# lawfuyang/HobbyRenderer

Hardware: AMD Instinct MI355X
Metric: Mrays/s at 1920×1080, 8 spp, 4 bounces; 1/2/4/8 GPU scaling (higher is better)
Workload: dtype f32; 1 GPU; config 2: Cornell-box-class procedural scene (38 triangles, 9 instances, closed room, emissive quad + default sun), 1920x1080, 8 spp (accumulation indices 0..7), 4 bounces; frames_in_flight=2, serial_kernels=False, mode=default

## Files before the change

hobbyrenderer_amd/csrc/pt_capi.cpp:

```cpp
#include <hip/hip_runtime.h>

#include <chrono>
#include <cstdio>
#include <cstdlib>
#include <cstring>
#include <mutex>
#include <new>
#include <stdexcept>
#include <limits>
#include <string>
#include <system_error>
#include <thread>
#include <vector>

#include "../../include/hobbyrt_pt.h"
#include "bvh_build.h"
#include "bvh_build_gpu.h"
#include "pt_device.h"
#include "pt_kernels.h"
#include "pt_motion.h"
#include "pt_wavefront.h"

using namespace hrt;

// ... 6 lines not shown
    std::vector<void*> bvhAllocations;
    GpuNodeQ* nodesQ = nullptr; size_t nodesQCapacity = 0;
    uint32_t nodes4Capacity = 0;
    GpuBvhBuilder* gpuBuilder = nullptr;
    GpuBvhBuilder* tlasBuilder = nullptr; uint32_t tlasBuilderInstances = 0;
    std::vector<HrptVertexQuantized> keptVertices; std::vector<uint32_t> keptIndices; std::vector<HrptMeshData> keptMeshData;
    std::vector<HrptPerInstanceData> keptInstances; std::vector<HrptMaterialConstants> keptMaterials; std::vector<HrptGPULight> keptLights;
    size_t lightCapacity = 0;
    SceneView view{};
    bool haveScene = false;
    uint32_t bvhNodes = 0, bvhTris = 0;
    uint32_t width = 0, height = 0;
    float4* dAccum = nullptr; float4* dOutput = nullptr; float4* dDisplay = nullptr;
    uint32_t* dHistogram = nullptr; float* dExposure = nullptr;
    uint32_t* dBloomDown = nullptr; uint32_t* dBloomUp = nullptr; size_t bloomWords = 0;
    uint32_t bloomTailTexels = 0;
    float4* dGBuffer[HRPT_GB_PLANES] = {};
    float4* dMotion = nullptr;
    MotionInst* dMotionInst = nullptr; size_t motionInstCapacity = 0;
    float* dMotionPositions = nullptr; uint32_t* dMotionIndices = nullptr;
    bool motionInstStale = true, motionGeometryStale = true;
    float4* dTemporal[2] = {}; int temporalCur = 0; bool temporalValid = false;
    float* dDenoiseTile = nullptr; float4* dDenoiseScratch[2] = {};
    DeviceCounters* dCounters = nullptr;
    hipEvent_t evStart = nullptr, evStop = nullptr;
    bool timed = false;
    WavefrontState wf;
    SceneTraits traits;
    int bvhBuilder = HRPT_BVH_BUILDER_AUTO;
    int accelStructure = HRPT_ACCEL_AUTO;
    BuiltTwoLevel* twoLevel = nullptr;
    std::vector<void*> meshAllocations;
    uint32_t megakernelFallbacks = 0;
    HrptBuildInfo buildInfo{};
};

static std::mutex g_errMutex;
static std::string g_createError;

static int fail(HrptContext* ctx, int code, const std::string& msg)
{
    if (ctx) ctx->err = msg;
    else { std::lock_guard<std::mutex> l(g_errMutex); g_createError = msg; }
    return code;
}
#define HIP_TRY(ctx, expr)                                                                         \
    do {                                                                                           \
        hipError_t e_ = (expr);                                                                    \
        if (e_ != hipSuccess) return fail(ctx, e_ == hipErrorOutOfMemory ? HRPT_ERR_OUT_OF_MEMORY : HRPT_ERR_HIP, \
                                          std::string(#expr) + ": " + hipGetErrorString(e_));      \
    } while (0)

static uint16_t float_to_half(float f)
{
    uint32_t x; memcpy(&x, &f, 4);
    uint32_t sign = (x >> 16) & 0x8000u;
    x &= 0x7fffffffu;
    if (x >= 0x47800000u) return (uint16_t)(sign | 0x7c00u | ((x > 0x7f800000u) ? (0x200u | ((x >> 13) & 0x3ffu)) : 0u));
    if (x < 0x38800000u) {
        if (x < 0x33000000u) return (uint16_t)sign;
        uint32_t shift = 126u - (x >> 23);
        uint32_t m = (x & 0x7fffffu) | 0x800000u;
        uint32_t h = m >> shift, rem = m & ((1u << shift) - 1u), halfway = 1u << (shift - 1u);
        if (rem > halfway || (rem == halfway && (h & 1u))) ++h;
        return (uint16_t)(sign | h);
    }
    uint32_t r = x + 0xfffu + ((x >> 13) & 1u);
    return (uint16_t)(sign | ((r - 0x38000000u) >> 13));
}

static void free_acceleration(HrptContext* c, bool keepGpuBuilder)
{
    for (void* p : c->bvhAllocations) (void)hipFree(p);
    c->bvhAllocations.clear();
    if (!keepGpuBuilder) {
        delete c->gpuBuilder; c->gpuBuilder = nullptr;
        delete c->tlasBuilder; c->tlasBuilder = nullptr; c->tlasBuilderInstances = 0;
        for (void* p : c->meshAllocations) (void)hipFree(p);
        c->meshAllocations.clear();
        delete c->twoLevel; c->twoLevel = nullptr;
    }
}

static void free_motion_tables(HrptContext* c)
{
    if (c->dMotionInst) (void)hipFree(c->dMotionInst);
    if (c->dMotionPositions) (void)hipFree(c->dMotionPositions);
    if (c->dMotionIndices) (void)hipFree(c->dMotionIndices);
    c->dMotionInst = nullptr; c->motionInstCapacity = 0; c->dMotionPositions = nullptr; c->dMotionIndices = nullptr;
    c->motionInstStale = c->motionGeometryStale = true;
}

static void free_scene(HrptContext* c)
{
    free_acceleration(c, false);
    free_motion_tables(c);
    for (void* p : c->allocations) (void)hipFree(p);
    c->allocations.clear();
    if (c->nodesQ) { (void)hipFree(c->nodesQ); c->nodesQ = nullptr; c->nodesQCapacity = 0; }
    c->keptVertices.clear(); c->keptIndices.clear(); c->keptMeshData.clear(); c->keptInstances.clear(); c->keptMaterials.clear(); c->keptLights.clear(); c->lightCapacity = 0;
    c->haveScene = false;
    memset(&c->view, 0, sizeof c->view);
}

template <class T>
static int upload(HrptContext* c, const T* host, size_t count, const T** dev, std::vector<void*>* owner = nullptr)
{
    *dev = nullptr;
    size_t bytes = count * sizeof(T);
    void* p = nullptr;
    HIP_TRY(c, hipMalloc(&p, bytes ? bytes : 16));
    (owner ? *owner : c->allocations).push_back(p);
    if (bytes) HIP_TRY(c, hipMemcpyAsync(p, host, bytes, hipMemcpyHostToDevice, c->stream));
    *dev = static_cast<const T*>(p);
    return HRPT_OK;
}

extern "C" {

int hrpt_create(const HrptDeviceDesc* desc, HrptContext** out)
{
    if (!desc || !out) return fail(nullptr, HRPT_ERR_INVALID_ARGUMENT, "hrpt_create: null argument");
    *out = nullptr;
    if (desc->abiVersion != HRPT_ABI_VERSION) return fail(nullptr, HRPT_ERR_INVALID_ARGUMENT, "hrpt_create: ABI version mismatch");
    int n = 0;
    hipError_t e = hipGetDeviceCount(&n);
    if (e != hipSuccess || n <= 0) return fail(nullptr, HRPT_ERR_NO_DEVICE, "hrpt_create: no HIP device available (the gfx950 kernels are the only backend)");
    if (desc->deviceOrdinal < 0 || desc->deviceOrdinal >= n) return fail(nullptr, HRPT_ERR_NO_DEVICE, "hrpt_create: device ordinal out of range");
    HrptContext* c = new HrptContext();
    c->device = desc->deviceOrdinal;
    if (hipSetDevice(c->device) != hipSuccess || hipStreamCreateWithFlags(&c->stream, hipStreamNonBlocking) != hipSuccess ||
        hipEventCreate(&c->evStart) != hipSuccess || hipEventCreate(&c->evStop) != hipSuccess ||
        hipMalloc((void**)&c->dCounters, sizeof(DeviceCounters) * kCounterShards) != hipSuccess ||
        hipMemset(c->dCounters, 0, sizeof(DeviceCounters) * kCounterShards) != hipSuccess) {
        int r = fail(nullptr, HRPT_ERR_HIP, "hrpt_create: stream/event/counter creation failed");
        delete c;
        return r;
    }
    c->ownStream = c->stream;
    if (const char* e = getenv("HRPT_WF_SEGMENT_SHIFT")) c->wf.knobs.segmentShift = (uint32_t)atoi(e);
    if (const char* e = getenv("HRPT_WF_SEGMENT_SIZE")) c->wf.knobs.segmentSize = (uint32_t)atoi(e);
    if (const char* e = getenv("HRPT_WF_BLOCKS_PER_CU")) c->wf.knobs.blocksPerCu = (uint32_t)atoi(e);
    if (const char* e = getenv("HRPT_WF_EXTEND_BLOCKS_PER_CU")) c->wf.knobs.extendBlocksPerCu = (uint32_t)atoi(e);
    if (const char* e = getenv("HRPT_WF_REFILL_MIN")) c->wf.knobs.refillMin = (uint32_t)atoi(e);
    if (const char* e = getenv("HRPT_WF_BVH_WIDTH")) c->wf.knobs.bvhWidth = (uint32_t)atoi(e);
    if (const char* e = getenv("HRPT_BVH_BUILDER")) c->bvhBuilder = (strcmp(e, "ploc") == 0 || strcmp(e, "2") == 0) ? HRPT_BVH_BUILDER_GPU_PLOC : ((strcmp(e, "gpu") == 0 || strcmp(e, "lbvh") == 0 || strcmp(e, "1") == 0) ? HRPT_BVH_BUILDER_GPU_LBVH : ((strcmp(e, "auto") == 0 || strcmp(e, "3") == 0) ? HRPT_BVH_BUILDER_AUTO : HRPT_BVH_BUILDER_HOST_SAH));
    if (const char* e = getenv("HRPT_WF_PAD_LDS")) c->wf.knobs.padLdsBytes = (uint32_t)atoi(e);
    if (const char* e = getenv("HRPT_WF_DRAIN_SEGMENTS")) c->wf.knobs.drainSegments = atoi(e) != 0;
    if (const char* e = getenv("HRPT_WF_SERIAL_SHADOW")) c->wf.knobs.serialShadow = atoi(e) != 0;
    if (const char* e = getenv("HRPT_WF_SHADOW_PATH")) c->wf.knobs.shadowPath = atoi(e);
    if (const char* e = getenv("HRPT_WF_SHADE_SORT")) c->wf.knobs.shadeSort = atoi(e) != 0 ? 1 : 0;
    if (const char* e = getenv("HRPT_WF_SLIM_SHADOW")) c->wf.knobs.noSlimShadow = atoi(e) == 0;
    if (const char* e = getenv("HRPT_WF_FUSED_PRIMARY")) c->wf.knobs.noFusedPrimary = atoi(e) == 0;
    if (const char* e = getenv("HRPT_WF_SHADE_LDS_TABLES")) c->wf.knobs.noShadeLdsTables = atoi(e) == 0;
    if (const char* e = getenv("HRPT_WF_NODE_LOOP_MIN")) c->wf.knobs.nodeLoopMin = (uint32_t)atoi(e);
    if (const char* e = getenv("HRPT_BLOOM_FUSED_TAIL")) { const int v = atoi(e); c->bloomTailTexels = v == 1 ? 8192u : (v > 0 ? (uint32_t)v : 0u); }
    *out = c;
    return HRPT_OK;
}

void hrpt_destroy(HrptContext* c)
{
    if (!c) return;
    (void)hipSetDevice(c->device);
    if (c->stream) (void)hipStreamSynchronize(c->stream);
    free_scene(c);
    wavefront_release(c->wf);
    if (c->dAccum) (void)hipFree(c->dAccum);
    if (c->dOutput) (void)hipFree(c->dOutput);
    if (c->dDisplay) (void)hipFree(c->dDisplay);
    for (float4* plane : c->dGBuffer) if (plane) (void)hipFree(plane);
    if (c->dMotion) (void)hipFree(c->dMotion);
    for (float4* image : c->dTemporal) if (image) (void)hipFree(image);
    for (float4* image : c->dDenoiseScratch) if (image) (void)hipFree(image);
    if (c->dDenoiseTile) (void)hipFree(c->dDenoiseTile);
    if (c->dHistogram) (void)hipFree(c->dHistogram);
    if (c->dExposure) (void)hipFree(c->dExposure);
    if (c->dBloomDown) (void)hipFree(c->dBloomDown);
    if (c->dBloomUp) (void)hipFree(c->dBloomUp);
    if (c->dCounters) (void)hipFree(c->dCounters);
    if (c->evStart) (void)hipEventDestroy(c->evStart);
    if (c->evStop) (void)hipEventDestroy(c->evStop);
    if (c->ownStream) (void)hipStreamDestroy(c->ownStream);
    delete c;
}

const char* hrpt_last_error(const HrptContext* c)
{
    if (c) return c->err.c_str();
    std::lock_guard<std::mutex> l(g_errMutex);
    static thread_local std::string copy;
    copy = g_createError;
    return copy.c_str();
}

static bool two_level_wanted(const HrptContext* c, const HrptSceneDesc& s, uint64_t sceneTris)
{
    int want = c->accelStructure;
    if (const char* e = getenv("HRPT_ACCEL_STRUCTURE")) { const int v = atoi(e); if (v >= HRPT_ACCEL_AUTO && v <= HRPT_ACCEL_TWO_LEVEL) want = v; }
    if (want == HRPT_ACCEL_FLAT || s.instanceCount == 0) return false;
    if (want == HRPT_ACCEL_TWO_LEVEL) return true;
    std::vector<uint8_t> used(s.meshDataCount, 0); uint32_t distinct = 0;
    for (uint32_t i = 0; i < s.instanceCount; ++i) if (!used[s.instances[i].m_MeshDataIndex]) { used[s.instances[i].m_MeshDataIndex] = 1; ++distinct; }
    bool nonOpaque = false;
    for (uint32_t i = 0; i < s.instanceCount && !nonOpaque; ++i) nonOpaque = s.materials[s.instances[i].m_MaterialIndex].m_AlphaMode != HRPT_ALPHA_MODE_OPAQUE;
    return sceneTris >= (nonOpaque ? (16ull << 20) : (2ull << 20)) && (uint64_t)s.instanceCount >= 8ull * distinct;
}

constexpr int kTwoLevelDoesNotFit = 1;
static bool build_instance_tree_on_gpu(HrptContext* c, uint32_t instanceCount, const std::vector<float>& boxes, bool rebuild, bool refit, GpuNode4* dstNodes, uint32_t& depth4Levels)
{
    std::string gerr;
    if (!c->tlasBuilder || c->tlasBuilderInstances != instanceCount) {
        delete c->tlasBuilder; c->tlasBuilder = new GpuBvhBuilder(); c->tlasBuilderInstances = 0;
        if (c->tlasBuilder->prepare_boxes(instanceCount, c->stream, gerr) != hipSuccess) { delete c->tlasBuilder; c->tlasBuilder = nullptr; return false; }
        c->tlasBuilderInstances = instanceCount;
    }
    GpuBuiltBvh g;
    bool ploc = c->bvhBuilder == HRPT_BVH_BUILDER_GPU_PLOC || (c->bvhBuilder != HRPT_BVH_BUILDER_GPU_LBVH && !rebuild);
    if (const char* e = getenv("HRPT_TLAS_LBVH")) ploc = atoi(e) == 0;
    const hipError_t ge = (rebuild && refit && c->tlasBuilder->can_refit()) ? c->tlasBuilder->refit_boxes(boxes.data(), c->stream, g, gerr)
                                                                              : c->tlasBuilder->build_boxes(boxes.data(), ploc, kTraversalStackDepth, c->stream, g, gerr);
    if (ge != hipSuccess || g.maxDepth + 2 > kTraversalStackDepth || g.node4Count == 0 || g.node4Count > instanceCount) return false;
    if (launch_tlas_fixup(g.nodes4, g.node4Count, g.leafOrder, dstNodes, c->stream) != hipSuccess || hipStreamSynchronize(c->stream) != hipSuccess) return false;
    depth4Levels = g.maxDepth4 + 1;
    c->buildInfo.deviceBuildMs = g.deviceMs; c->buildInfo.usedBuilder = (g.ploc ? HRPT_BVH_BUILDER_GPU_PLOC : HRPT_BVH_BUILDER_GPU_LBVH) | (g.refitted ? HRPT_BVH_BUILDER_REFITTED : 0u);
    return true;
}

static int build_two_level(HrptContext* c, const HrptSceneDesc& s, SceneView& v, bool instancesOnly, bool refit)
{
    std::string berr; int r;
    const bool timing = getenv("HRPT_BUILD_TIMING") != nullptr; auto tp = std::chrono::steady_clock::now();
    auto lap = [&](const char* what) { if (!timing) return; (void)hipStreamSynchronize(c->stream); auto t = std::chrono::steady_clock::now(); fprintf(stderr, "[two-level] %-22s %7.3f ms\n", what, std::chrono::duration<float, std::milli>(t - tp).count()); tp = t; };
    bool gpuTree = s.instanceCount >= 1024 && c->bvhBuilder != HRPT_BVH_BUILDER_HOST_SAH;
    if (const char* e = getenv("HRPT_TLAS_BUILDER")) gpuTree = s.instanceCount >= 8 && (strcmp(e, "gpu") == 0 || strcmp(e, "1") == 0);
    lap("(entry)");
    std::vector<float> boxes;
    std::vector<float>* wantBoxes = gpuTree ? &boxes : nullptr;
    if (!instancesOnly) { delete c->twoLevel; c->twoLevel = new BuiltTwoLevel(); }
    if (!(instancesOnly ? rebuild_two_level_instances(s, *c->twoLevel, berr, wantBoxes) : build_scene_two_level(s, *c->twoLevel, berr, wantBoxes))) {
        if (berr.find("singular") != std::string::npos) return kTwoLevelDoesNotFit;
        return fail(c, HRPT_ERR_INVALID_ARGUMENT, "acceleration structure: " + berr);
    }
    lap("host records");
    BuiltTwoLevel& b = *c->twoLevel;
    if (two_level_stack_need(b) > 128u) return kTwoLevelDoesNotFit;
    if (!instancesOnly) {
        const HostTri* dt; const HostTriAttr* da; const HostTriTangent* dtg;
        if ((r = upload(c, b.tris.data(), b.tris.size(), &dt, &c->meshAllocations)) != HRPT_OK) return r;
        if ((r = upload(c, b.attrs.data(), b.attrs.size(), &da, &c->meshAllocations)) != HRPT_OK) return r;
        v.tris = reinterpret_cast<const GpuTri*>(dt); v.triCount = (uint32_t)b.tris.size(); v.attrs = reinterpret_cast<const GpuTriAttr*>(da);
        v.tangents = nullptr;
        if (!b.tangents.empty()) {
            if ((r = upload(c, b.tangents.data(), b.tangents.size(), &dtg, &c->meshAllocations)) != HRPT_OK) return r;
            v.tangents = reinterpret_cast<const GpuTriTangent*>(dtg);
        }
    }
    const HostNode4* dn4; const HostInstance* di; const HostInstShade* dis;
    if (b.nodes4.size() >= kMaxStructureNodes) return fail(c, HRPT_ERR_INVALID_ARGUMENT, "acceleration structure: more than 2^25 nodes (32-bit node offsets in the traversal kernels)");
    if (gpuTree) {
        void* p = nullptr;
        HIP_TRY(c, hipMalloc(&p, b.nodes4.size() * sizeof(HostNode4)));
        c->bvhAllocations.push_back(p);
        dn4 = static_cast<const HostNode4*>(p);
        HIP_TRY(c, hipMemcpyAsync(static_cast<HostNode4*>(p) + b.tlasNodeCount, b.nodes4.data() + b.tlasNodeCount, (b.nodes4.size() - b.tlasNodeCount) * sizeof(HostNode4), hipMemcpyHostToDevice, c->stream));
    } else if ((r = upload(c, b.nodes4.data(), b.nodes4.size(), &dn4, &c->bvhAllocations)) != HRPT_OK) return r;
    if ((r = upload(c, b.instances.data(), b.instances.size(), &di, &c->bvhAllocations)) != HRPT_OK) return r;
    if ((r = upload(c, b.instShade.data(), b.instShade.size(), &dis, &c->bvhAllocations)) != HRPT_OK) return r;
    lap("uploads");
    if (gpuTree) {
        uint32_t levels = 0;
        if (build_instance_tree_on_gpu(c, s.instanceCount, boxes, instancesOnly, refit, const_cast<GpuNode4*>(reinterpret_cast<const GpuNode4*>(dn4)), levels)) {
            b.maxDepth4Tlas = levels;
        } else {
            for (void* p : c->bvhAllocations) (void)hipFree(p);
            c->bvhAllocations.clear();
            if (!rebuild_two_level_instances(s, b, berr)) return fail(c, HRPT_ERR_INVALID_ARGUMENT, "acceleration structure: " + berr);
            if ((r = upload(c, b.nodes4.data(), b.nodes4.size(), &dn4, &c->bvhAllocations)) != HRPT_OK) return r;
            if ((r = upload(c, b.instances.data(), b.instances.size(), &di, &c->bvhAllocations)) != HRPT_OK) return r;
            if ((r = upload(c, b.instShade.data(), b.instShade.size(), &dis, &c->bvhAllocations)) != HRPT_OK) return r;
            gpuTree = false;
        }
    }
    lap("instance tree (GPU)");
    if (two_level_stack_need(b) > 128u) return kTwoLevelDoesNotFit;
    v.nodes = nullptr; v.nodeCount = b.tlasNodeCount; v.rootLeaf = b.tlasRootLeaf;
    v.nodes4 = reinterpret_cast<const GpuNode4*>(dn4); v.node4Count = (uint32_t)b.nodes4.size(); v.nodesQ = nullptr;
    v.instances = reinterpret_cast<const GpuInstance*>(di); v.instanceCount = (uint32_t)b.instances.size();
    v.instShade = reinterpret_cast<const GpuInstShade*>(dis);
    HIP_TRY(c, hipStreamSynchronize(c->stream));
    if (!gpuTree) c->buildInfo.usedBuilder = HRPT_BVH_BUILDER_HOST_SAH;
    c->buildInfo.structure = HRPT_ACCEL_TWO_LEVEL;
    c->buildInfo.instanceNodeCount = b.tlasNodeCount; c->buildInfo.distinctMeshes = b.distinctMeshes;
    c->buildInfo.triangleCount = v.triCount; c->buildInfo.nodeCount = 0; c->buildInfo.node4Count = v.node4Count;
    c->buildInfo.maxDepth = 0; c->buildInfo.maxDepth4 = b.maxDepth4Tlas + b.maxDepth4Blas;
    c->bvhNodes = v.node4Count; c->bvhTris = v.triCount;
    c->traits.bvhMaxDepth = 0; c->traits.bvh4MaxDepth = b.maxDepth4Tlas + b.maxDepth4Blas; c->traits.twoLevelStackNeed = two_level_stack_need(b); c->traits.quantisedNodes = false;
    return HRPT_OK;
}

static int build_acceleration(HrptContext* c, const HrptSceneDesc& s, uint64_t sceneTris, SceneView& v, bool firstBuild, bool refit = false)
{
    const auto t0 = std::chrono::steady_clock::now();
    std::string berr;
    int r;
// ... 624 lines not shown

int hrpt_resolve_device(HrptContext* c, const float* accumulationDevice, float* outputDevice, uint64_t pixelCount, void* stream)
{
    if (!c) return HRPT_ERR_INVALID_ARGUMENT;
    if (!accumulationDevice || !outputDevice) return fail(c, HRPT_ERR_INVALID_ARGUMENT, "hrpt_resolve_device: null image");
    if (pixelCount == 0) return HRPT_OK;
    if (pixelCount > 0xFFFFFFFFull) return fail(c, HRPT_ERR_INVALID_ARGUMENT, "hrpt_resolve_device: image too large");
    HIP_TRY(c, hipSetDevice(c->device));
    HIP_TRY(c, launch_resolve(reinterpret_cast<const float4*>(accumulationDevice), reinterpret_cast<float4*>(outputDevice), (uint32_t)pixelCount,
                              static_cast<hipStream_t>(stream)));
    return HRPT_OK;
}

int hrpt_allgather(HrptContext* const* ranks, int n)
{
    if (!ranks || n <= 0) return HRPT_ERR_INVALID_ARGUMENT;
    for (int i = 0; i < n; ++i) if (!ranks[i]) return HRPT_ERR_INVALID_ARGUMENT;
    HrptContext* c0 = ranks[0];
    const uint32_t W = c0->width, H = c0->height;
    if (!c0->dAccum || W == 0 || H == 0) return fail(c0, HRPT_ERR_INVALID_ARGUMENT, "hrpt_allgather: hrpt_resize not called");
    if (H % (uint32_t)n != 0) return fail(c0, HRPT_ERR_INVALID_ARGUMENT, "hrpt_allgather: image height must be a multiple of the number of ranks");
    for (int i = 0; i < n; ++i) {
        if (ranks[i]->width != W || ranks[i]->height != H || !ranks[i]->dAccum) return fail(c0, HRPT_ERR_INVALID_ARGUMENT, "hrpt_allgather: contexts differ in image size");
        for (int j = 0; j < i; ++j) if (ranks[j] == ranks[i]) return fail(c0, HRPT_ERR_INVALID_ARGUMENT, "hrpt_allgather: the same context appears twice");
    }
    const size_t rows = H / (uint32_t)n, bandBytes = rows * (size_t)W * sizeof(float4);
    std::vector<hipEvent_t> sent((size_t)n, nullptr);
    auto cleanup = [&]() { for (hipEvent_t e : sent) if (e) (void)hipEventDestroy(e); };
    for (int i = 0; i < n; ++i) {
        HrptContext* src = ranks[i];
        hipError_t e = hipSetDevice(src->device);
        if (e == hipSuccess) e = hipEventCreateWithFlags(&sent[(size_t)i], hipEventDisableTiming);
        const size_t off = (size_t)i * rows * W;
        for (int j = 0; j < n && e == hipSuccess; ++j) {
            if (j == i) continue;
            HrptContext* dst = ranks[j];
            hipEvent_t ready = nullptr;
            e = hipSetDevice(dst->device);
            if (e == hipSuccess) e = hipEventCreateWithFlags(&ready, hipEventDisableTiming);
            if (e == hipSuccess) e = hipEventRecord(ready, dst->stream);
            if (e == hipSuccess) e = hipSetDevice(src->device);
            if (e == hipSuccess) e = hipStreamWaitEvent(src->stream, ready, 0);
            if (e == hipSuccess) e = hipMemcpyPeerAsync(dst->dAccum + off, dst->device, src->dAccum + off, src->device, bandBytes, src->stream);
            if (ready) (void)hipEventDestroy(ready);
        }
        if (e == hipSuccess) e = hipEventRecord(sent[(size_t)i], src->stream);
        if (e != hipSuccess) { cleanup(); return fail(c0, HRPT_ERR_HIP, std::string("hrpt_allgather (send): ") + hipGetErrorString(e)); }
    }
    for (int j = 0; j < n; ++j) {
        HrptContext* dst = ranks[j];
        hipError_t e = hipSetDevice(dst->device);
        for (int i = 0; i < n && e == hipSuccess; ++i) if (i != j) e = hipStreamWaitEvent(dst->stream, sent[(size_t)i], 0);
        if (e == hipSuccess) e = launch_resolve(dst->dAccum, dst->dOutput, W * H, dst->stream);
        if (e != hipSuccess) { cleanup(); return fail(c0, HRPT_ERR_HIP, std::string("hrpt_allgather (receive): ") + hipGetErrorString(e)); }
    }
    cleanup();
    return HRPT_OK;
}

int hrpt_trace_rays(HrptContext* c, const HrptRay* rays, HrptRayHit* hits, uint64_t count, uint32_t flags)
{
    if (!c) return HRPT_ERR_INVALID_ARGUMENT;
    if (!c->haveScene) return fail(c, HRPT_ERR_INVALID_ARGUMENT, "hrpt_trace_rays: no scene uploaded");
    if (count == 0) return HRPT_OK;
    if (!rays || !hits) return fail(c, HRPT_ERR_INVALID_ARGUMENT, "hrpt_trace_rays: null array");
    if ((flags & 0xFFu) > HRPT_RAYS_SHADOW || (flags & ~(0xFFu | HRPT_RAYS_DEVICE_POINTERS | HRPT_RAYS_THREAD_PER_RAY))) return fail(c, HRPT_ERR_INVALID_ARGUMENT, "hrpt_trace_rays: unknown flags");
    if (count > (1ull << 31)) return fail(c, HRPT_ERR_INVALID_ARGUMENT, "hrpt_trace_rays: too many rays in one call");
    if (c->view.instances && ((flags & HRPT_RAYS_THREAD_PER_RAY) || !wavefront_trace_rays_supported(c->traits)) && c->traits.twoLevelStackNeed > 64u)
        return fail(c, HRPT_ERR_INVALID_ARGUMENT, "hrpt_trace_rays: this two-level structure is deeper than the thread-per-ray kernel's 64-entry stack");
    HIP_TRY(c, hipSetDevice(c->device));
    const bool shadow = (flags & 0xFFu) == HRPT_RAYS_SHADOW;
    const bool persistent = !(flags & HRPT_RAYS_THREAD_PER_RAY) && wavefront_trace_rays_supported(c->traits) && c->view.node4Count > 0;
    auto trace = [&](const HrptRay* dr, HrptRayHit* dh) -> hipError_t {
        if (!persistent) return launch_trace_rays(c->view, dr, dh, count, shadow, c->stream);
        std::string werr;
        hipError_t te = wavefront_trace_rays(c->wf, c->view, c->traits, dr, dh, count, shadow, c->stream, werr);
        if (te != hipSuccess) c->err = "hrpt_trace_rays: " + werr;
        return te;
    };
    if (flags & HRPT_RAYS_DEVICE_POINTERS) {
        HIP_TRY(c, trace(rays, hits));
        return HRPT_OK;
    }
    HrptRay* dRays = nullptr; HrptRayHit* dHits = nullptr;
    hipError_t e = hipMalloc(reinterpret_cast<void**>(&dRays), count * sizeof(HrptRay));
    if (e == hipSuccess) e = hipMalloc(reinterpret_cast<void**>(&dHits), count * sizeof(HrptRayHit));
    if (e == hipSuccess) e = hipMemcpyAsync(dRays, rays, count * sizeof(HrptRay), hipMemcpyHostToDevice, c->stream);
    if (e == hipSuccess) e = trace(dRays, dHits);
    if (e == hipSuccess) e = hipMemcpyAsync(hits, dHits, count * sizeof(HrptRayHit), hipMemcpyDeviceToHost, c->stream);
    if (e == hipSuccess) e = hipStreamSynchronize(c->stream);
    if (dRays) (void)hipFree(dRays);
    if (dHits) (void)hipFree(dHits);
    if (e != hipSuccess) return fail(c, e == hipErrorOutOfMemory ? HRPT_ERR_OUT_OF_MEMORY : HRPT_ERR_HIP, std::string("hrpt_trace_rays: ") + hipGetErrorString(e));
    return HRPT_OK;
}

int hrpt_resolve_columns_device(HrptContext* c, const float* shardsDevice, float* accumulationDevice, float* outputDevice, uint32_t width, uint32_t height, uint32_t ranks, void* stream)
{
    if (!c) return HRPT_ERR_INVALID_ARGUMENT;
    if (!shardsDevice || !outputDevice) return fail(c, HRPT_ERR_INVALID_ARGUMENT, "hrpt_resolve_columns_device: null image");
    if (ranks == 0 || width == 0 || height == 0 || width % (8u * ranks) != 0) return fail(c, HRPT_ERR_INVALID_ARGUMENT, "hrpt_resolve_columns_device: width must be a positive multiple of 8 * ranks");
    if ((uint64_t)width * height > 0xFFFFFFFFull) return fail(c, HRPT_ERR_INVALID_ARGUMENT, "hrpt_resolve_columns_device: image too large");
    HIP_TRY(c, hipSetDevice(c->device));
    HIP_TRY(c, launch_resolve_columns(reinterpret_cast<const float4*>(shardsDevice), reinterpret_cast<float4*>(accumulationDevice), reinterpret_cast<float4*>(outputDevice),
                                      width, height, ranks, static_cast<hipStream_t>(stream)));
    return HRPT_OK;
}

int hrpt_set_shadow_overlap(HrptContext* c, int enabled)
{
    if (!c) return HRPT_ERR_INVALID_ARGUMENT;
    c->wf.knobs.serialShadow = enabled == 0;
    return HRPT_OK;
}

int hrpt_set_acceleration_structure(HrptContext* c, int structure)
{
    if (!c) return HRPT_ERR_INVALID_ARGUMENT;
    if (structure < HRPT_ACCEL_AUTO || structure > HRPT_ACCEL_TWO_LEVEL) return fail(c, HRPT_ERR_INVALID_ARGUMENT, "hrpt_set_acceleration_structure: unknown structure");
    c->accelStructure = structure;
    return HRPT_OK;
}

int hrpt_set_bvh_builder(HrptContext* c, int builder)
{
    if (!c) return HRPT_ERR_INVALID_ARGUMENT;
    if (builder != HRPT_BVH_BUILDER_HOST_SAH && builder != HRPT_BVH_BUILDER_GPU_LBVH && builder != HRPT_BVH_BUILDER_GPU_PLOC && builder != HRPT_BVH_BUILDER_AUTO) return fail(c, HRPT_ERR_INVALID_ARGUMENT, "hrpt_set_bvh_builder: unknown builder");
    c->bvhBuilder = builder;
    return HRPT_OK;
}

int hrpt_get_build_info(HrptContext* c, HrptBuildInfo* out)
{
    if (!c) return HRPT_ERR_INVALID_ARGUMENT;
    if (!out) return fail(c, HRPT_ERR_INVALID_ARGUMENT, "hrpt_get_build_info: null out");
    if (!c->haveScene) return fail(c, HRPT_ERR_INVALID_ARGUMENT, "hrpt_get_build_info: no scene uploaded");
    *out = c->buildInfo;
    return HRPT_OK;
}

int hrpt_get_stats(HrptContext* c, HrptStats* out)
{
    if (!c) return HRPT_ERR_INVALID_ARGUMENT;
    if (!out) return fail(c, HRPT_ERR_INVALID_ARGUMENT, "hrpt_get_stats: null out");
    HIP_TRY(c, hipSetDevice(c->device));
    HIP_TRY(c, hipStreamSynchronize(c->stream));
    DeviceCounters h[kCounterShards];
    HIP_TRY(c, hipMemcpy(h, c->dCounters, sizeof h, hipMemcpyDeviceToHost));
    memset(out, 0, sizeof *out);
    DeviceCounters total{};
    for (int i = 0; i < kCounterShards; ++i) {
        total.closestRays += h[i].closestRays; total.shadowRays += h[i].shadowRays; total.paths += h[i].paths; total.neeEntries += h[i].neeEntries;
        total.neeSamples += h[i].neeSamples; total.radianceShade += h[i].radianceShade; total.radianceShadow += h[i].radianceShadow; total.skipped16 += h[i].skipped16;
    }
    out->closestRays = total.closestRays; out->shadowRays = total.shadowRays; out->paths = total.paths;
    out->neeEntries = total.neeEntries; out->neeSamples = total.neeSamples;
    out->megakernelFallbacks = c->megakernelFallbacks; out->queuePoolBytes = c->wf.poolBytes;
    if (total.neeEntries || c->wf.raygenBytes || c->wf.resolveBytes) {
        wavefront_queue_bytes(c->wf, total, out->traceQueueBytes, out->shadeQueueBytes, out->shadowQueueBytes);
        out->raygenQueueBytes = c->wf.raygenBytes; out->resolveQueueBytes = c->wf.resolveBytes;
    }
    if (c->timed) { float ms = 0.0f; if (hipEventElapsedTime(&ms, c->evStart, c->evStop) == hipSuccess) out->lastRenderMs = ms; }
    wavefront_collect_timing(c->wf);
    out->traceKernelMs = c->wf.kernelMs[0]; out->traceKernelLaunches = c->wf.kernelLaunches[0];
    out->shadeKernelMs = c->wf.kernelMs[1]; out->shadeKernelLaunches = c->wf.kernelLaunches[1];
    out->shadowKernelMs = c->wf.kernelMs[2]; out->shadowKernelLaunches = c->wf.kernelLaunches[2];
    out->raygenKernelMs = c->wf.kernelMs[3]; out->raygenKernelLaunches = c->wf.kernelLaunches[3];
    out->resolveKernelMs = c->wf.kernelMs[4]; out->resolveKernelLaunches = c->wf.kernelLaunches[4];
    out->bvhNodeCount = c->bvhNodes; out->bvhTriangleCount = c->bvhTris; out->bvhMaxDepth = c->traits.bvhMaxDepth;
    return HRPT_OK;
}

int hrpt_post_process(HrptContext* c, const HrptPostParams* p)
{
    if (!c) return HRPT_ERR_INVALID_ARGUMENT;
    if (!p) return fail(c, HRPT_ERR_INVALID_ARGUMENT, "hrpt_post_process: null params");
    if (!c->dOutput) return fail(c, HRPT_ERR_INVALID_ARGUMENT, "hrpt_post_process: hrpt_resize not called");
    HIP_TRY(c, hipSetDevice(c->device));
    if (!c->dExposure) {
        HIP_TRY(c, hipMalloc((void**)&c->dExposure, 16));
        HIP_TRY(c, hipMalloc((void**)&c->dHistogram, 256 * sizeof(uint32_t)));
        const float one[4] = { 1.0f, 0.0f, 0.0f, 0.0f };
        HIP_TRY(c, hipMemcpy(c->dExposure, one, 16, hipMemcpyHostToDevice));
    }
    if (!c->dDisplay) HIP_TRY(c, hipMalloc((void**)&c->dDisplay, (size_t)c->width * c->height * sizeof(float4)));
    HIP_TRY(c, launch_post_chain(c->dOutput, c->dDisplay, c->width * c->height, *p, c->dHistogram, c->dExposure, c->stream));
    return HRPT_OK;
}

static int bloom_run(HrptContext* c, float4* image, uint32_t width, uint32_t height, const HrptBloomParams& p, hipStream_t stream)
{
    const size_t words = bloom_pyramid_words(width, height);
    if (words == 0) return HRPT_OK;
    if (words != c->bloomWords) {
        if (c->dBloomDown) { (void)hipFree(c->dBloomDown); c->dBloomDown = nullptr; }
        if (c->dBloomUp) { (void)hipFree(c->dBloomUp); c->dBloomUp = nullptr; }
        c->bloomWords = 0;
        HIP_TRY(c, hipMalloc((void**)&c->dBloomDown, words * sizeof(uint32_t)));
        HIP_TRY(c, hipMalloc((void**)&c->dBloomUp, words * sizeof(uint32_t)));
        c->bloomWords = words;
    }
    HIP_TRY(c, launch_bloom(image, width, height, p, c->dBloomDown, c->dBloomUp, c->bloomTailTexels, stream));
    return HRPT_OK;
}

int hrpt_bloom(HrptContext* c, const HrptBloomParams* p)
{
    if (!c) return HRPT_ERR_INVALID_ARGUMENT;
    if (!p) return fail(c, HRPT_ERR_INVALID_ARGUMENT, "hrpt_bloom: null params");
    if (!bloom_params_valid(*p)) return fail(c, HRPT_ERR_INVALID_ARGUMENT, "hrpt_bloom: knee, intensity and upsampleRadius must be finite and >= 0");
    if (!c->dOutput) return fail(c, HRPT_ERR_INVALID_ARGUMENT, "hrpt_bloom: hrpt_resize not called");
    HIP_TRY(c, hipSetDevice(c->device));
    return bloom_run(c, c->dOutput, c->width, c->height, *p, c->stream);
}

int hrpt_bloom_device(HrptContext* c, float* hdrDevice, uint32_t width, uint32_t height, const HrptBloomParams* p, void* stream)
{
    if (!c) return HRPT_ERR_INVALID_ARGUMENT;
    if (!p) return fail(c, HRPT_ERR_INVALID_ARGUMENT, "hrpt_bloom_device: null params");
    if (!hdrDevice) return fail(c, HRPT_ERR_INVALID_ARGUMENT, "hrpt_bloom_device: null image");
    if (width == 0 || height == 0 || width > 65535u || height > 65535u) return fail(c, HRPT_ERR_INVALID_ARGUMENT, "hrpt_bloom_device: size must be 1..65535");
    if (!bloom_params_valid(*p)) return fail(c, HRPT_ERR_INVALID_ARGUMENT, "hrpt_bloom_device: knee, intensity and upsampleRadius must be finite and >= 0");
    HIP_TRY(c, hipSetDevice(c->device));
    return bloom_run(c, reinterpret_cast<float4*>(hdrDevice), width, height, *p, static_cast<hipStream_t>(stream));
}

int hrpt_bloom_host(const float* hdrIn, float* hdrOut, uint32_t width, uint32_t height, const HrptBloomParams* p, int nthreads)
{
    if (!p) return fail(nullptr, HRPT_ERR_INVALID_ARGUMENT, "hrpt_bloom_host: null params");
    if (!hdrIn || !hdrOut) return fail(nullptr, HRPT_ERR_INVALID_ARGUMENT, "hrpt_bloom_host: null image");
    if (width == 0 || height == 0 || width > 65535u || height > 65535u) return fail(nullptr, HRPT_ERR_INVALID_ARGUMENT, "hrpt_bloom_host: size must be 1..65535");
    if (!bloom_params_valid(*p)) return fail(nullptr, HRPT_ERR_INVALID_ARGUMENT, "hrpt_bloom_host: knee, intensity and upsampleRadius must be finite and >= 0");
    if (nthreads <= 0) { nthreads = (int)std::thread::hardware_concurrency(); if (nthreads > 16) nthreads = 16; }
    if (nthreads < 1) nthreads = 1;
    if (nthreads > 256) nthreads = 256;
    try { bloom_host(hdrIn, hdrOut, width, height, *p, nthreads); }
    catch (const std::bad_alloc&) { return fail(nullptr, HRPT_ERR_OUT_OF_MEMORY, "hrpt_bloom_host: out of memory"); }
    catch (const std::system_error& e) { return fail(nullptr, HRPT_ERR_UNSUPPORTED, std::string("hrpt_bloom_host: ") + e.what()); }
    return HRPT_OK;
}

int hrpt_bloom_pack_probe(const float* rgb, uint32_t count, uint32_t* packed, float* unpackedRgb)
{
    if (!rgb && count) return fail(nullptr, HRPT_ERR_INVALID_ARGUMENT, "hrpt_bloom_pack_probe: null input");
    bloom_pack_probe(rgb, count, packed, unpackedRgb);
    return HRPT_OK;
}

static int temporal_check(HrptContext* c, const char* what, const HrptTemporalImages* img, uint32_t width, uint32_t height, const HrptPlanarViewConstants* view,
                          const HrptPlanarViewConstants* prevView, const HrptTemporalParams* p)
{
    const std::string w(what);
    if (!img || !view || !prevView || !p) return fail(c, HRPT_ERR_INVALID_ARGUMENT, w + ": null argument");
    if (!img->color || !img->motion || !img->depth || !img->normal || !img->historyOut || !img->colorOut)
        return fail(c, HRPT_ERR_INVALID_ARGUMENT, w + ": null image (only historyIn may be NULL)");
    if (img->historyOut == img->historyIn) return fail(c, HRPT_ERR_INVALID_ARGUMENT, w + ": historyOut must differ from historyIn");
    if (width == 0 || height == 0 || width > 65535u || height > 65535u) return fail(c, HRPT_ERR_INVALID_ARGUMENT, w + ": size must be 1..65535");
    if (!(view->m_ViewportSize[0] == (float)width && view->m_ViewportSize[1] == (float)height))
        return fail(c, HRPT_ERR_INVALID_ARGUMENT, w + ": view->m_ViewportSize does not match the image size");
    if (!temporal_params_valid(*p)) return fail(c, HRPT_ERR_INVALID_ARGUMENT, w + ": blend must be finite and in [0, 1], flags HRPT_TEMPORAL_* only, reserved 0");
    return HRPT_OK;
}

int hrpt_temporal_host(const HrptTemporalImages* img, uint32_t width, uint32_t height, const HrptPlanarViewConstants* view,
                       const HrptPlanarViewConstants* prevView, const HrptTemporalParams* p, int nthreads)
{
    int r = temporal_check(nullptr, "hrpt_temporal_host", img, width, height, view, prevView, p);
    if (r != HRPT_OK) return r;
    if (nthreads <= 0) { nthreads = (int)std::thread::hardware_concurrency(); if (nthreads > 16) nthreads = 16; }
    if (nthreads < 1) nthreads = 1;
    if (nthreads > 256) nthreads = 256;
    try { temporal_host(*img, width, height, *view, *prevView, *p, nthreads); }
    catch (const std::bad_alloc&) { return fail(nullptr, HRPT_ERR_OUT_OF_MEMORY, "hrpt_temporal_host: out of memory"); }
    catch (const std::system_error& e) { return fail(nullptr, HRPT_ERR_UNSUPPORTED, std::string("hrpt_temporal_host: ") + e.what()); }
    return HRPT_OK;
}

int hrpt_temporal_device(HrptContext* c, const HrptTemporalImages* img, uint32_t width, uint32_t height, const HrptPlanarViewConstants* view,
                         const HrptPlanarViewConstants* prevView, const HrptTemporalParams* p, void* stream)
{
    if (!c) return HRPT_ERR_INVALID_ARGUMENT;
    int r = temporal_check(c, "hrpt_temporal_device", img, width, height, view, prevView, p);
    if (r != HRPT_OK) return r;
    HIP_TRY(c, hipSetDevice(c->device));
    HIP_TRY(c, launch_temporal(*img, width, height, *view, *prevView, *p, static_cast<hipStream_t>(stream)));
    return HRPT_OK;
}

int hrpt_temporal_accumulate(HrptContext* c, const HrptPlanarViewConstants* view, const HrptPlanarViewConstants* prevView, const HrptTemporalParams* p)
{
    if (!c) return HRPT_ERR_INVALID_ARGUMENT;
    if (!view || !prevView || !p) return fail(c, HRPT_ERR_INVALID_ARGUMENT, "hrpt_temporal_accumulate: null argument");
    if (!c->dOutput) return fail(c, HRPT_ERR_INVALID_ARGUMENT, "hrpt_temporal_accumulate: hrpt_resize not called");
    if (!c->dMotion || !c->dGBuffer[HRPT_GB_DEPTH] || !c->dGBuffer[HRPT_GB_NORMAL])
        return fail(c, HRPT_ERR_INVALID_ARGUMENT, "hrpt_temporal_accumulate: the motion, depth or normal plane was never requested (hrpt_render_motion_vectors with planeMask = DEPTH | NORMAL fills them)");
    HIP_TRY(c, hipSetDevice(c->device));
    const size_t bytes = (size_t)c->width * c->height * sizeof(float4);
    const bool fresh = !c->dTemporal[0];
    const int next = fresh ? 0 : 1 - c->temporalCur;
    HrptTemporalImages img{};
    img.color = reinterpret_cast<const float*>(c->dOutput); img.colorOut = reinterpret_cast<float*>(c->dOutput);
    img.motion = reinterpret_cast<const float*>(c->dMotion);
    img.depth = reinterpret_cast<const float*>(c->dGBuffer[HRPT_GB_DEPTH]); img.normal = reinterpret_cast<const float*>(c->dGBuffer[HRPT_GB_NORMAL]);
    img.historyOut = reinterpret_cast<float*>(c->dOutput);
    int r = temporal_check(c, "hrpt_temporal_accumulate", &img, c->width, c->height, view, prevView, p);
    if (r != HRPT_OK) return r;
// ... 309 lines not shown
```

hobbyrenderer_amd/csrc/pt_kernels.h:

```cpp
#pragma once

#include <hip/hip_runtime.h>
#include <stdint.h>

#include "../../include/hobbyrt_pt.h"

namespace hrt {

struct SceneView;
struct MotionArgs;
struct GpuNode4; struct GpuNodeQ;

constexpr int kCounterShards = 32;
struct DeviceCounters {
    unsigned long long closestRays;
    unsigned long long shadowRays;
    unsigned long long paths;
    unsigned long long neeEntries;
    unsigned long long neeSamples;
    unsigned long long radianceShade;
    unsigned long long radianceShadow;
    unsigned long long skipped16;
};

struct TileRect {
    uint32_t x0, y0, x1, y1;
    uint32_t stripeCount = 1, stripeIndex = 0;
    __host__ __device__ uint32_t columns() const { uint32_t all = (x1 - x0 + 7u) / 8u; return all > stripeIndex ? (all - stripeIndex + stripeCount - 1u) / stripeCount : 0u; }
    __host__ __device__ uint32_t column_x(uint32_t k) const { return x0 + (k * stripeCount + stripeIndex) * 8u; }
};

hipError_t launch_megakernel(const SceneView& scene, const HrptPathTracerConstants& constants, float4* accumulation,
                             float4* output, uint32_t imageWidth, TileRect rect, DeviceCounters* counters, hipStream_t stream);

hipError_t launch_gbuffer_megakernel(const SceneView& scene, const HrptPathTracerConstants& constants, float4* const* planes, uint32_t planeMask,
                                     uint32_t imageWidth, TileRect rect, hipStream_t stream);

hipError_t launch_motion_megakernel(const SceneView& scene, const HrptPathTracerConstants& constants, float4* const* planes, uint32_t planeMask,
                                    const MotionArgs& motion, uint32_t imageWidth, TileRect rect, hipStream_t stream);

hipError_t launch_post_chain(const float4* hdr, float4* display, uint32_t pixelCount, const HrptPostParams& params, uint32_t* histogram,
                             float* exposure, hipStream_t stream);

size_t bloom_pyramid_words(uint32_t width, uint32_t height);
bool bloom_params_valid(const HrptBloomParams& params);
hipError_t launch_bloom(float4* hdr, uint32_t width, uint32_t height, const HrptBloomParams& params, uint32_t* downPyramid, uint32_t* upPyramid,
                        uint32_t tailTexels, hipStream_t stream);
void bloom_pack_probe(const float* rgb, uint32_t count, uint32_t* packed, float* unpacked);
void bloom_host(const float* hdrIn, float* hdrOut, uint32_t width, uint32_t height, const HrptBloomParams& params, int nthreads);

bool temporal_params_valid(const HrptTemporalParams& params);
hipError_t launch_temporal(const HrptTemporalImages& images, uint32_t width, uint32_t height, const HrptPlanarViewConstants& view,
                           const HrptPlanarViewConstants& prevView, const HrptTemporalParams& params, hipStream_t stream);
void temporal_host(const HrptTemporalImages& images, uint32_t width, uint32_t height, const HrptPlanarViewConstants& view,
                   const HrptPlanarViewConstants& prevView, const HrptTemporalParams& params, int nthreads);

bool denoise_params_valid(const HrptDenoiseParams& params);
size_t denoise_noise_floats();
void denoise_default_tile(float* tile);
hipError_t launch_denoise(const HrptDenoiseImages& images, uint32_t width, uint32_t height, const HrptPlanarViewConstants& view,
                          const HrptDenoiseParams& params, float radius, uint32_t frame, hipStream_t stream);
void denoise_host(const HrptDenoiseImages& images, uint32_t width, uint32_t height, const HrptPlanarViewConstants& view,
                  const HrptDenoiseParams& params, int nthreads);

hipError_t launch_trace_rays(const SceneView& scene, const HrptRay* rays, HrptRayHit* hits, uint64_t count, bool shadow, hipStream_t stream);

hipError_t launch_quantise_nodes(const GpuNode4* nodes4, uint32_t count, GpuNodeQ* out, double* leafArea, hipStream_t stream);
hipError_t launch_bvh_check(const SceneView& scene, unsigned long long* violations, hipStream_t stream);
hipError_t launch_unorm8_table(float* out512, hipStream_t stream);
hipError_t launch_f16_table(float* out, hipStream_t stream);
hipError_t launch_sample_textures(const SceneView& scene, uint32_t materialCount, const HrptTextureProbe* probes, HrptTextureProbeResult* results,
                                  uint32_t count, hipStream_t stream);

hipError_t launch_resolve(const float4* accumulation, float4* output, uint32_t pixelCount, hipStream_t stream);
hipError_t launch_resolve_columns(const float4* shards, float4* accumulation, float4* output, uint32_t width, uint32_t height, uint32_t ranks, hipStream_t stream);

}
```

hobbyrenderer_amd/csrc/pt_wavefront.h:

```cpp
#pragma once

#include <hip/hip_runtime.h>
#include <stdint.h>
#include <string>
#include <vector>

#include "../../include/hobbyrt_pt.h"
#include "pt_kernels.h"
#include "pt_wavefront_plan.h"

namespace hrt {

struct SceneView;
struct MotionArgs;

struct WavefrontState {
    void* pool = nullptr;
    size_t poolBytes = 0;
    void* spill = nullptr;
    size_t spillBytes = 0;
    void* traceSpill = nullptr;
    size_t traceSpillBytes = 0;
    void* gbPool = nullptr;
    size_t gbPoolBytes = 0;
    std::vector<hipEvent_t> events;
    std::vector<uint8_t> kind;
    uint32_t eventsUsed = 0;
    float kernelMs[5] = { 0.0f, 0.0f, 0.0f, 0.0f, 0.0f };
    uint32_t kernelLaunches[5] = { 0, 0, 0, 0, 0 };
    uint64_t raygenBytes = 0, resolveBytes = 0;
    RenderPlan plan;
    uint32_t shadeInstances = 0, shadeMaterials = 0;
    WavefrontKnobs knobs;
    bool profile = false;
    hipStream_t auxStream = nullptr;
    std::vector<hipEvent_t> forkEvents, joinEvents;
};

bool wavefront_supports(const SceneView& scene, const HrptPathTracerConstants& constants);
hipError_t wavefront_render(WavefrontState& st, const SceneView& scene, const SceneTraits& traits, const HrptPathTracerConstants& constants,
                            uint32_t accumCount, float4* accumulation, float4* output, uint32_t width, uint32_t height, TileRect rect,
                            DeviceCounters* counters, hipStream_t stream, std::string& error);
hipError_t wavefront_trace_rays(WavefrontState& st, const SceneView& scene, const SceneTraits& traits, const HrptRay* rays, HrptRayHit* hits, uint64_t count,
                                bool shadow, hipStream_t stream, std::string& error);
hipError_t wavefront_gbuffer(WavefrontState& st, const SceneView& scene, const SceneTraits& traits, const HrptPathTracerConstants& constants,
                             float4* const* planes, uint32_t planeMask, uint32_t width, TileRect rect, hipStream_t stream, std::string& error,
                             const MotionArgs* motion = nullptr);
void wavefront_release(WavefrontState& st);
void wavefront_collect_timing(WavefrontState& st);
void wavefront_reset_timing(WavefrontState& st);
void wavefront_queue_bytes(const WavefrontState& st, const DeviceCounters& total, uint64_t& trace, uint64_t& shade, uint64_t& shadow);

}
```

hobbyrenderer_amd/csrc/pt_wavefront.hip:

```cpp
#define HRPT_PHASE_TU 1
#include "pt_wavefront.h"

#include <mutex>
#include <type_traits>
#include <unordered_map>
#include <vector>

#include "bvh_build.h"
#include "pt_gbuffer.h"
#include "pt_motion.h"
#include "pt_path.h"

#ifdef HRPT_PHASE_PROFILE
__device__ unsigned long long g_phaseCounters[128];
#endif
#ifdef HRPT_SKY_DEBUG
__device__ float g_skyDebug[2048 * 16];
#endif

namespace hrt {

namespace {

constexpr uint32_t kMaxSppPerBatch = 64;
// ... 457 lines not shown
    const uint32_t wavesPerBlock = kBlock / 64;
    const uint32_t gw = uniform(blockIdx.x * wavesPerBlock + (threadIdx.x >> 6)), totalWaves = gridDim.x * wavesPerBlock;
    TlCull tl; tl.inv = mk3(0.0f, 0.0f, 0.0f); tl.noi = tl.inv; tl.noiF = tl.inv; tl.inst = -1;
    const uint64_t numChunks = (a.count + (1u << kTraceChunkShift) - 1) >> kTraceChunkShift;
    const bool emptyScene = s.nodeCount == 0 && s.rootLeaf == 0;

    uint64_t chunk = gw; uint32_t cnt = 0, next = 0; uint64_t chunkBase = 0; bool haveChunk = false;
    auto open_chunk = [&]() {
        haveChunk = chunk < numChunks; next = 0;
        if (haveChunk) { chunkBase = chunk << kTraceChunkShift; const uint64_t left = a.count - chunkBase; cnt = left < (1u << kTraceChunkShift) ? (uint32_t)left : (1u << kTraceChunkShift); }
    };
    open_chunk();
    bool active = false;
    Ray r; r.o = mk3(0.0f, 0.0f, 0.0f); r.d = mk3(0.0f, 0.0f, 1.0f); r.tmin = 0.0f; r.tmax = 1e10f;
    RayShear sh = make_shear(r.d); f3 inv = mk3(0.0f, 0.0f, 0.0f), noi = mk3(0.0f, 0.0f, 0.0f);
    HitKey lower; lower.have = false; lower.t = 0.0f; lower.inst = 0; lower.prim = 0;
    Hit best; best.valid = false; best.t = 0.0f; best.inst = 0; best.prim = 0; best.u = 0.0f; best.v = 0.0f; best.opaque = 0; best.tri = 0;
    int32_t cur = kTraversalDone; int sp = 0; uint64_t slot = 0; uint32_t rng = 0; float tlim = 0.0f;
    bool blocked = false, candOverflow = false, finite = true; int candCount = 0;
    for (;;) {
        if (haveChunk && next >= cnt) { chunk += totalWaves; open_chunk(); }
        const unsigned long long mIdle = __ballot(!active);
        const uint32_t nIdle = (uint32_t)__popcll(mIdle);
        if (haveChunk && (nIdle >= a.refillMin || nIdle == 64u)) {
            const uint32_t idx = next + prefix_rank(mIdle);
            if (!active && idx < cnt) {
                slot = chunkBase + idx;
                const float4* rp = reinterpret_cast<const float4*>(a.rays + slot);
                const float4 q0 = rp[0], q1 = rp[1]; const uint32_t rr = reinterpret_cast<const uint32_t*>(rp + 2)[0];
                const f3 o = mk3(q0.x, q0.y, q0.z), d = mk3(q1.x, q1.y, q1.z);
                finite = d.x == d.x && d.y == d.y && d.z == d.z && o.x == o.x && o.y == o.y && o.z == o.z;
                if (SHADOW) r = shadow_ray(o, d, q1.w);
                else { r.o = o; r.d = d; r.tmin = q0.w; r.tmax = q1.w; }
                rng = rr; blocked = false; candOverflow = false; candCount = 0; lower.have = false; best.valid = false; tlim = r.tmax; sp = 0;
                sh = make_shear(r.d);
                if constexpr (TL) tl_world(tl, r); else { inv = traversal_rcp(r.d); noi = slab_origin_term(r.o, inv); }
                cur = (emptyScene || !finite) ? kTraversalDone : (s.nodeCount == 0 ? s.rootLeaf : 0);
                active = true;
            }
            next += nIdle;
        }
        if (__ballot(active) == 0ull) { if (haveChunk) continue; break; }
        if (active) {
            if constexpr (TL) {
                while (cur >= 0 && cur != kExitBlas) {
                    cur = inner_step(gbvh, cur, tl.noi, tl.noiF, tl.inv, r.tmin, tlim, stack, sp);
                    if ((uint32_t)__popcll(__ballot(cur >= 0 && cur != kExitBlas)) < a.nodeLoopMin) break;
                }
                if (cur == kExitBlas || (cur < 0 && cur != kTraversalDone && tl.inst < 0)) cur = tl_switch(gbvh, cur, tl, r, stack, sp);
                else if (cur < 0 && cur != kTraversalDone) {
                    const GpuInstance& I = s.instances[tl.inst];
                    const uint32_t enc = (uint32_t)(~cur), first = enc >> 2, count = (enc & 3u) + 1u, inst = (uint32_t)tl.inst;
                    for (uint32_t i = 0; i < count; ++i) {
                        float4 ta, tb, tc; gbvh.tri(first + i, ta, tb, tc);
                        f3 p0, p1, p2; tl_world_triangle(I, ta, tb, tc, p0, p1, p2);
                        float t, u, v;
                        const bool hitTri = tri_test(p0, p1, p2, r, sh, t, u, v);
                        if (SHADOW) { if (hitTri) { if (I.flags & 1u) { blocked = true; break; } candCount = 1; } continue; }
                        const uint32_t prim = __float_as_uint(tb.w);
                        const bool ok = !lower.have || key_less(lower.t, lower.inst, lower.prim, t, inst, prim);
                        const bool take = hitTri && ok && (!best.valid || key_less(t, inst, prim, best.t, best.inst, best.prim));
                        best.t = take ? t : best.t; best.u = take ? u : best.u; best.v = take ? v : best.v;
                        best.inst = take ? inst : best.inst; best.prim = take ? prim : best.prim; best.tri = take ? first + i : best.tri;
                        best.valid = best.valid || take; best.opaque = take ? (I.flags & 1u) : best.opaque;
                        tlim = take ? t : tlim;
                    }
                    cur = blocked ? kTraversalDone : stack.pop(--sp);
                }
            } else {
            while (cur >= 0) {
                if (LDS_BVH) cur = inner_step(lbvh, cur, noi, inv, r.tmin, tlim, stack, sp);
                else cur = inner_step(gbvh, cur, noi, inv, r.tmin, tlim, stack, sp);
                if ((uint32_t)__popcll(__ballot(cur >= 0)) < a.nodeLoopMin) break;
            }
            if (cur < 0 && cur != kTraversalDone) {
                const uint32_t enc = (uint32_t)(~cur), first = enc >> 2, count = (enc & 3u) + 1u;
                for (uint32_t i = 0; i < count; ++i) {
                    float4 ta, tb, tc;
                    if (LDS_BVH) lbvh.tri(first + i, ta, tb, tc); else gbvh.tri(first + i, ta, tb, tc);
                    float t, u, v;
                    if (tri_test(mk3(ta.x, ta.y, ta.z), mk3(tb.x, tb.y, tb.z), mk3(tc.x, tc.y, tc.z), r, sh, t, u, v)) {
                        if (SHADOW) {
                            if (__float_as_uint(tc.w) & 1u) { blocked = true; break; }
                            if (LDS_BVH) candidate_insert<kShadowCandidates>(lbvh, cand, candCount, candOverflow, t, first + i, __float_as_uint(ta.w), __float_as_uint(tb.w));
                            else candidate_insert<kShadowCandidates>(gbvh, cand, candCount, candOverflow, t, first + i, __float_as_uint(ta.w), __float_as_uint(tb.w));
                            continue;
                        }
                        const uint32_t inst = __float_as_uint(ta.w), prim = __float_as_uint(tb.w);
                        const bool ok = !lower.have || key_less(lower.t, lower.inst, lower.prim, t, inst, prim);
                        const bool take = ok && (!best.valid || key_less(t, inst, prim, best.t, best.inst, best.prim));
                        best.t = take ? t : best.t; best.u = take ? u : best.u; best.v = take ? v : best.v;
                        best.inst = take ? inst : best.inst; best.prim = take ? prim : best.prim; best.tri = take ? first + i : best.tri;
                        best.opaque = take ? (__float_as_uint(tc.w) & 1u) : best.opaque;
                        best.valid = best.valid || take;
                        tlim = take ? t : tlim;
                    }
                }
                cur = (blocked || sp == 0) ? kTraversalDone : stack.pop(--sp);
            }
            }
            if (cur == kTraversalDone) {
                HrptRayHit out; out.t = 0.0f; out.u = 0.0f; out.v = 0.0f; out.instance = 0; out.primitive = 0; out.hit = 0; out.rng = rng; out.pad = 0;
                bool done = true;
                if (SHADOW) {
                    float vis = 1.0f;
                    if (finite) {
                        if (blocked) vis = 0.0f;
                        else if (candCount > 0) {
                            if constexpr (TL) vis = shadow_retrace_two_level(s, gbvh, r, stack);
                            else if (LDS_BVH) vis = shadow_resolve_candidates(s, lbvh, r, sh, candCount, candOverflow, cand, stack);
                            else vis = shadow_resolve_candidates(s, gbvh, r, sh, candCount, candOverflow, cand, stack);
                        }
                    }
                    out.t = vis; out.hit = vis < 1.0f ? 1u : 0u;
                } else if (best.valid && !best.opaque && !candidate_commits(s, best, rng)) {
                    lower.have = true; lower.t = best.t; lower.inst = best.inst; lower.prim = best.prim;
                    best.valid = false; tlim = r.tmax; sp = 0;
                    cur = s.nodeCount == 0 ? s.rootLeaf : 0;
                    if constexpr (TL) tl_world(tl, r);
                    done = false;
                } else if (best.valid) { out.t = best.t; out.u = best.u; out.v = best.v; out.instance = best.inst; out.primitive = best.prim; out.hit = 1u; out.rng = rng; }
                if (done) {
                    out.rng = rng;
                    float4* hp = reinterpret_cast<float4*>(a.hits + slot);
                    hp[0] = make_float4(out.t, out.u, out.v, __uint_as_float(out.instance));
                    hp[1] = make_float4(__uint_as_float(out.primitive), __uint_as_float(out.hit), __uint_as_float(out.rng), 0.0f);
                    active = false;
                }
            }
        }
    }
}

template <int MAXL>
struct NeeBuf { float ux[MAXL], uy[MAXL]; uint32_t light[MAXL]; };

HRT_DEV LdsShadeTables copy_shade_tables(char* dst, const WfArgs& a)
{
    const SceneView& s = a.scene;
    const uint32_t nA = s.triCount * (uint32_t)(sizeof(GpuTriAttr) / 16), nI = a.shadeInstances * (uint32_t)(sizeof(GpuInstShade) / 16);
    const uint32_t nM = a.shadeMaterials * (uint32_t)(sizeof(HrptMaterialConstants) / 4);
    float4* const dA = reinterpret_cast<float4*>(dst); float4* const dI = dA + nA; uint32_t* const dM = reinterpret_cast<uint32_t*>(dI + nI);
    const float4* const sA = reinterpret_cast<const float4*>(s.attrs); const float4* const sI = reinterpret_cast<const float4*>(s.instShade);
    const uint32_t* const sM = reinterpret_cast<const uint32_t*>(s.materials);
    for (uint32_t i = threadIdx.x; i < nA; i += kBlock) dA[i] = sA[i];
    for (uint32_t i = threadIdx.x; i < nI; i += kBlock) dI[i] = sI[i];
    for (uint32_t i = threadIdx.x; i < nM; i += kBlock) dM[i] = sM[i];
    LdsShadeTables t;
    t.attrs = (uint32_t)(uintptr_t)(LdsShadeTables::LdsPtr)dst; t.instShade = t.attrs + nA * 16u; t.materials = t.instShade + nI * 16u;
    return t;
}


template <int MAXL, bool SIMPLE, bool PRIMARY, bool LDS_TABLES>
HRT_DEV void shade_paths(const WfArgs& a, const HrptPathTracerConstants& cb, uint32_t parity, int bounce, int lastBounce)
{
    static_assert(!PRIMARY || SIMPLE, "no raygen pass: SIMPLE scenes only");
    static_assert(!LDS_TABLES || SIMPLE, "tables in LDS: behind the ring of the SIMPLE variants");
    const uint32_t wavesPerBlock = kBlock / 64, lane = lane_id();
    const uint32_t gw = uniform(blockIdx.x * wavesPerBlock + (threadIdx.x >> 6)), totalWaves = gridDim.x * wavesPerBlock;
    const uint32_t in = parity, out = parity ^ 1u;
    const SceneView& s = a.scene;
    extern __shared__ __attribute__((aligned(16))) char shadeSmem[];
    constexpr uint32_t kRing = kShadeRing, kRingFields = kShadeRingFields;
    float* const ring = reinterpret_cast<float*>(shadeSmem) + (size_t)uniform(threadIdx.x >> 6) * kRing * kRingFields;
    LdsShadeTables ldsTables; ldsTables.attrs = ldsTables.instShade = ldsTables.materials = 0u;
    if constexpr (LDS_TABLES) { ldsTables = copy_shade_tables(shadeSmem + kShadeRingBytes, a); __syncthreads(); }
    const GlobalShadeTables globalTables{ s };
    auto shade_hit = [&](PathState& ps, const Hit& h, SurfaceCarry& carry, auto&& emit) {
        if constexpr (LDS_TABLES) return shade_surface_a<!SIMPLE, !SIMPLE, SIMPLE>(s, ldsTables, cb, ps, h, carry, emit);
        else return shade_surface_a<!SIMPLE, !SIMPLE, SIMPLE>(s, globalTables, cb, ps, h, carry, emit);
    };
    uint32_t ringHead = 0, pending = 0;
    unsigned int nEntriesOut = 0, nRadiance = 0;
    constexpr bool SORT = !SIMPLE;
    const uint32_t segSize = a.segSize;
    uint16_t* const permBase = reinterpret_cast<uint16_t*>(shadeSmem) + (size_t)uniform(threadIdx.x >> 6) * segSize * 2;
    uint8_t* const keys = reinterpret_cast<uint8_t*>(shadeSmem) + (size_t)wavesPerBlock * segSize * 4 + (size_t)uniform(threadIdx.x >> 6) * segSize;
    uint32_t permSel = 0;
    bool permuted = false, permutedB = false;
    auto sort_segment = [&](uint32_t base, uint32_t n, uint16_t* perm) -> bool {
        HRT_PHASE(PH_SHADE_SORT);
        uint32_t c0 = 0, c1 = 0, c2 = 0;
        for (uint32_t b = 0; b < n; b += 64) {
            const uint32_t e = b + lane; uint32_t k = 4u;
            if (e < n) { k = __float_as_uint(a.b.hit[base + e].w) >> 29; k = k > 3u ? 3u : k; keys[e] = (uint8_t)k; }
            c0 += (uint32_t)__popcll(__ballot(k == 0u)); c1 += (uint32_t)__popcll(__ballot(k == 1u)); c2 += (uint32_t)__popcll(__ballot(k == 2u));
        }
        const uint32_t c3 = n - c0 - c1 - c2;
        if (c0 == n || c1 == n || c2 == n || c3 == n) return false;
        __builtin_amdgcn_fence(__ATOMIC_SEQ_CST, "wavefront");
        uint32_t b0 = 0, b1 = c0, b2 = c0 + c1, b3 = c0 + c1 + c2;
        for (uint32_t b = 0; b < n; b += 64) {
            const uint32_t e = b + lane; const uint32_t k = e < n ? keys[e] : 4u;
            const unsigned long long m0 = __ballot(k == 0u), m1 = __ballot(k == 1u), m2 = __ballot(k == 2u), m3 = __ballot(k == 3u);
            if (k == 0u) perm[b0 + prefix_rank(m0)] = (uint16_t)e;
            if (k == 1u) perm[b1 + prefix_rank(m1)] = (uint16_t)e;
            if (k == 2u) perm[b2 + prefix_rank(m2)] = (uint16_t)e;
            if (k == 3u) perm[b3 + prefix_rank(m3)] = (uint16_t)e;
            b0 += (uint32_t)__popcll(m0); b1 += (uint32_t)__popcll(m1); b2 += (uint32_t)__popcll(m2); b3 += (uint32_t)__popcll(m3);
        }
        __builtin_amdgcn_fence(__ATOMIC_SEQ_CST, "wavefront");
        return true;
    };
    {
        uint32_t seg = gw, cnt = 0, segBase = 0, next = 0, outCount = 0, shCount = 0;
        bool haveSeg = false;
        auto open_segment = [&]() {
            haveSeg = false; cnt = 0; next = 0; outCount = 0; shCount = 0;
            for (; seg < a.numSegments; seg += totalWaves) {
                cnt = uniform(PRIMARY ? path_count(a, in, seg) : a.b.pathCnt[in][seg]);
                if (cnt) { segBase = seg * a.segSize; haveSeg = true; break; }
                if (lane == 0) { a.b.pathCnt[out][seg] = 0; a.b.shadowCnt[seg] = 0; }
            }
            if (SORT && a.sortShade && haveSeg) permuted = sort_segment(segBase, cnt, permBase + permSel * segSize);
        };
        open_segment();
        while (haveSeg) {
            const uint32_t takeA = cnt - next < 64u ? cnt - next : 64u;
            const uint32_t segA = seg, baseA = segBase, nextA = next;
            const bool endsA = nextA + takeA >= cnt;
            uint32_t takeB = 0, segB = 0, baseB = 0, cntB = 0;
            if (endsA && takeA < 64u) {
                uint32_t probe = seg + totalWaves;
                for (; probe < a.numSegments; probe += totalWaves) {
                    cntB = uniform(PRIMARY ? path_count(a, in, probe) : a.b.pathCnt[in][probe]);
                    if (cntB) break;
                    if (lane == 0) { a.b.pathCnt[out][probe] = 0; a.b.shadowCnt[probe] = 0; }
                }
                if (probe < a.numSegments) {
                    segB = probe; baseB = probe * a.segSize; takeB = cntB < 64u - takeA ? cntB : 64u - takeA;
                    if (SORT && a.sortShade) permutedB = sort_segment(baseB, cntB, permBase + (permSel ^ 1u) * segSize);
                } else segB = probe;
            }
            const bool inA = lane < takeA;
            uint32_t outCountB = 0, shCountB = 0;
            bool valid = lane < takeA + takeB, alive = false, wantDefer = false, wantRadiance = false;
            LobeDraw ld; ld.spec = false; ld.specProb = 0.0f; ld.root = 0.0f; ld.sp = 0.0f; ld.cp = 0.0f;
            uint32_t nNee = 0, smp = 0, slotIn = 0;
            PathState ps; f3 neeT = mk3(0.0f, 0.0f, 0.0f);
            constexpr bool STREAMED = MAXL == 0;
            NeeBuf<(STREAMED ? 1 : MAXL)> nee; SurfaceCarry carry;
            if (valid) {
                HRT_PHASE(PH_SHADE_ITER);
                uint32_t slot = inA ? baseA + ((SORT && permuted) ? (uint32_t)permBase[permSel * segSize + nextA + lane] : nextA + lane)
                                    : baseB + ((SORT && permutedB) ? (uint32_t)permBase[(permSel ^ 1u) * segSize + (lane - takeA)] : lane - takeA);
                slotIn = slot;
                float4 o, d, t;
                if constexpr (PRIMARY) {
                    const PrimaryArgs& pr = *a.primaryArgs;
                    o = make_float4(pr.cam[0], pr.cam[1], pr.cam[2], 0.0f); d = a.b.rayD[in][slot];
                    t = make_float4(1.0f, 1.0f, 1.0f, __uint_as_float(slot));
                } else { o = a.b.rayO[in][slot]; d = a.b.rayD[in][slot]; t = a.b.thr[in][slot]; }
                float4 ha = a.b.hit[slot]; uint32_t tri = __float_as_uint(ha.w);
                const bool noPath = PRIMARY && tri == kNoPathRecord;
                if (tri < kNoPathRecord) tri &= 0x1FFFFFFFu;
                ps.ray.o = mk3(o.x, o.y, o.z); ps.ray.d = mk3(d.x, d.y, d.z); ps.ray.tmin = o.w; ps.ray.tmax = 1e10f;
                ps.rng = __float_as_uint(d.w);
                ps.throughput = mk3(t.x, t.y, t.z); smp = __float_as_uint(t.w);
                ps.radiance = mk3(0.0f, 0.0f, 0.0f);
                if (!SIMPLE && a.hasMedium) {
                    float4 m0 = a.b.med0[in][slot], m1 = a.b.med1[in][slot];
                    ps.sigmaA = mk3(m0.x, m0.y, m0.z); ps.interiorIOR = m0.w; ps.sigmaS = mk3(m1.x, m1.y, m1.z); ps.inVolume = m1.w != 0.0f;
                } else { ps.sigmaA = mk3(0.0f, 0.0f, 0.0f); ps.sigmaS = mk3(0.0f, 0.0f, 0.0f); ps.interiorIOR = 1.0f; ps.inVolume = false; }
                bool addRadiance = false; f3 add = mk3(0.0f, 0.0f, 0.0f);
                if (noPath) {
                } else if (tri != 0xFFFFFFFFu) {
                    HRT_PHASE(PH_SHADE_HIT);
                    Hit h; h.valid = true; h.t = ha.x; h.u = ha.y; h.v = ha.z; h.tri = tri; h.prim = 0; h.inst = s.instances ? a.b.hitInst[slot] : 0u; h.opaque = 1;
                    f3 emissiveTerm = mk3(0.0f, 0.0f, 0.0f);
                    SurfaceOutcome oc = shade_hit(ps, h, carry, [&](uint32_t li, float ux, float uy) {
                        if (STREAMED) ++nNee;
                        else if (nNee < (uint32_t)MAXL) { nee.ux[nNee] = ux; nee.uy[nNee] = uy; nee.light[nNee] = li; ++nNee; }
                    });
                    if (oc == SURFACE_TRANSMITTED) alive = true;
                    else {
                        emissiveTerm = ps.radiance;
                        if (emissiveTerm.x != 0.0f || emissiveTerm.y != 0.0f || emissiveTerm.z != 0.0f) { addRadiance = true; add = emissiveTerm; }
                        neeT = ps.throughput;
                        if (!lastBounce) {
                            if (SIMPLE) {
                                if (lobe_begin(ps, carry, bounce, ld)) {
                                    if (ld.spec) wantDefer = true;
                                    else alive = lobe_diffuse(ps, carry.worldPos, carry.N, carry.baseColor, carry.metallic, ld);
                                }
                            } else alive = shade_surface_b(ps, carry, bounce);
                        }
                    }
                } else {
                    miss_sky(s, cb, ps, bounce);
                    addRadiance = true; add = ps.radiance;
#ifdef HRPT_SKY_DEBUG
                    if (smp < 2048u && bounce == 0) {
                        float* g = g_skyDebug + smp * 16u;
                        g[0] = ps.ray.o.x; g[1] = ps.ray.o.y; g[2] = ps.ray.o.z; g[3] = ps.ray.d.x; g[4] = ps.ray.d.y; g[5] = ps.ray.d.z;
                        g[6] = cb.m_SunDirection[0]; g[7] = cb.m_SunDirection[1]; g[8] = cb.m_SunDirection[2]; g[9] = s.lights[0].m_Intensity;
                        g[10] = ps.radiance.x; g[11] = ps.radiance.y; g[12] = ps.radiance.z; g[13] = ps.throughput.x; g[14] = ps.throughput.y; g[15] = ps.throughput.z;
                    }
#endif
                }
                if constexpr (PRIMARY) {
                    a.b.radiance[smp] = addRadiance ? make_float4(0.0f + add.x, 0.0f + add.y, 0.0f + add.z, 0.0f) : make_float4(0.0f, 0.0f, 0.0f, 0.0f);
                } else if (addRadiance) {
                    float4 r = a.b.radiance[smp];
                    r.x = r.x + add.x; r.y = r.y + add.y; r.z = r.z + add.z;
                    a.b.radiance[smp] = r;
                }
                if (lastBounce) alive = false;
                wantRadiance = addRadiance && !PRIMARY;
            }
            nRadiance += (unsigned int)__popcll(__ballot(wantRadiance));
            const unsigned long long mA = __ballot(alive && inA), mB = __ballot(alive && !inA);
            if (alive) {
                HRT_PHASE(PH_SHADE_WRITE);
                uint32_t o = inA ? baseA + outCount + prefix_rank(mA) : baseB + prefix_rank(mB);
                a.b.rayO[out][o] = make_float4(ps.ray.o.x, ps.ray.o.y, ps.ray.o.z, ps.ray.tmin);
                a.b.rayD[out][o] = make_float4(ps.ray.d.x, ps.ray.d.y, ps.ray.d.z, __uint_as_float(ps.rng));
                a.b.thr[out][o] = make_float4(ps.throughput.x, ps.throughput.y, ps.throughput.z, __uint_as_float(smp));
                if (!SIMPLE && a.hasMedium) {
                    a.b.med0[out][o] = make_float4(ps.sigmaA.x, ps.sigmaA.y, ps.sigmaA.z, ps.interiorIOR);
                    a.b.med1[out][o] = make_float4(ps.sigmaS.x, ps.sigmaS.y, ps.sigmaS.z, ps.inVolume ? 1.0f : 0.0f);
                }
            }
            const unsigned long long msA = __ballot(nNee > 0 && inA), msB = __ballot(nNee > 0 && !inA);
            if (SIMPLE && MAXL == 1 && a.slimShadow && nNee > 0) {
                uint32_t e = inA ? baseA + shCount + prefix_rank(msA) : baseB + prefix_rank(msB);
                a.b.sh0[e] = make_float4(carry.worldPos.x, carry.worldPos.y, carry.worldPos.z, __uint_as_float(slotIn));
                a.b.sh1[e] = make_float4(carry.N.x, carry.N.y, carry.N.z, __uint_as_float(carry.material));
            } else if (nNee > 0) {
                uint32_t e = inA ? baseA + shCount + prefix_rank(msA) : baseB + prefix_rank(msB);
                a.b.sh0[e] = make_float4(carry.worldPos.x, carry.worldPos.y, carry.worldPos.z, __uint_as_float(smp));
                a.b.sh1[e] = make_float4(carry.N.x, carry.N.y, carry.N.z, carry.roughness);
                a.b.sh2[e] = make_float4(carry.V.x, carry.V.y, carry.V.z, carry.metallic);
                a.b.sh3[e] = make_float4(carry.baseColor.x, carry.baseColor.y, carry.baseColor.z, carry.ior);
                a.b.sh4[e] = make_float4(neeT.x, neeT.y, neeT.z, __uint_as_float(nNee));
                if (STREAMED) {
                    const f3 sunDir = mk3(cb.m_SunDirection[0], cb.m_SunDirection[1], cb.m_SunDirection[2]);
                    uint32_t rng = carry.rngBeforeLights, j = 0;
                    for (uint32_t i = 0; i < cb.m_LightCount; ++i) {
                        HrptGPULight l = load_light(s, i);
                        float ux, uy;
                        if (nee_draw<false>(l, carry.N, carry.worldPos, sunDir, rng, ux, uy)) a.b.shL[(size_t)e * a.maxLights + j++] = make_float4(ux, uy, __uint_as_float(i), 0.0f);
                    }
                } else {
#pragma unroll
                    for (int j = 0; j < (STREAMED ? 1 : MAXL); ++j)
                        if ((uint32_t)j < nNee) a.b.shL[(size_t)e * a.maxLights + j] = make_float4(nee.ux[j], nee.uy[j], __uint_as_float(nee.light[j]), 0.0f);
                }
            }
            outCount += (uint32_t)__popcll(mA); shCount += (uint32_t)__popcll(msA);
            outCountB = (uint32_t)__popcll(mB); shCountB = (uint32_t)__popcll(msB);
            nEntriesOut += (unsigned int)(__popcll(msA) + __popcll(msB));
            if (SIMPLE) {
                const unsigned long long md = __ballot(wantDefer);
                const uint32_t nNew = (uint32_t)__popcll(md);
                bool parked = false;
                for (int round = 0; round < 2 && !parked; ++round) {
                parked = pending + nNew <= kRing;
                if (parked && wantDefer) {
                    float* e = ring + ((ringHead + pending + prefix_rank(md)) & (kRing - 1u));
                    e[0 * kRing] = carry.N.x; e[1 * kRing] = carry.N.y; e[2 * kRing] = carry.N.z;
                    e[3 * kRing] = carry.V.x; e[4 * kRing] = carry.V.y; e[5 * kRing] = carry.V.z;
                    e[6 * kRing] = carry.F0.x; e[7 * kRing] = carry.F0.y; e[8 * kRing] = carry.F0.z;
                    e[9 * kRing] = carry.roughness; e[10 * kRing] = ld.root; e[11 * kRing] = ld.sp; e[12 * kRing] = ld.cp; e[13 * kRing] = ld.specProb;
                    e[14 * kRing] = carry.worldPos.x; e[15 * kRing] = carry.worldPos.y; e[16 * kRing] = carry.worldPos.z;
                    e[17 * kRing] = ps.throughput.x; e[18 * kRing] = ps.throughput.y; e[19 * kRing] = ps.throughput.z;
                    e[20 * kRing] = __uint_as_float(ps.rng); e[21 * kRing] = __uint_as_float(smp); e[22 * kRing] = inA ? 1.0f : 0.0f;
                }
                if (parked) pending += nNew;
                __builtin_amdgcn_fence(__ATOMIC_SEQ_CST, "wavefront");
                while (pending >= 64u || ((endsA || !parked) && pending)) {
                    const uint32_t n = pending < 64u ? pending : 64u;
                    bool alive2 = false, tagA = true; PathState q; uint32_t smp2 = 0;
                    if (lane < n) {
                        const float* e = ring + ((ringHead + lane) & (kRing - 1u));
                        f3 N = mk3(e[0 * kRing], e[1 * kRing], e[2 * kRing]), V = mk3(e[3 * kRing], e[4 * kRing], e[5 * kRing]), F0 = mk3(e[6 * kRing], e[7 * kRing], e[8 * kRing]);
                        LobeDraw d2; d2.spec = true; d2.root = e[10 * kRing]; d2.sp = e[11 * kRing]; d2.cp = e[12 * kRing]; d2.specProb = e[13 * kRing];
                        f3 wp = mk3(e[14 * kRing], e[15 * kRing], e[16 * kRing]);
                        q.throughput = mk3(e[17 * kRing], e[18 * kRing], e[19 * kRing]); q.rng = __float_as_uint(e[20 * kRing]); smp2 = __float_as_uint(e[21 * kRing]);
                        tagA = e[22 * kRing] != 0.0f;
                        alive2 = lobe_specular(q, wp, N, V, F0, e[9 * kRing], d2);
                    }
                    const unsigned long long m2A = __ballot(alive2 && tagA), m2B = __ballot(alive2 && !tagA);
                    if (alive2) {
                        uint32_t o = tagA ? baseA + outCount + prefix_rank(m2A) : baseB + outCountB + prefix_rank(m2B);
                        a.b.rayO[out][o] = make_float4(q.ray.o.x, q.ray.o.y, q.ray.o.z, q.ray.tmin);
                        a.b.rayD[out][o] = make_float4(q.ray.d.x, q.ray.d.y, q.ray.d.z, __uint_as_float(q.rng));
                        a.b.thr[out][o] = make_float4(q.throughput.x, q.throughput.y, q.throughput.z, __uint_as_float(smp2));
                    }
                    outCount += (uint32_t)__popcll(m2A); outCountB += (uint32_t)__popcll(m2B);
                    ringHead = (ringHead + n) & (kRing - 1u); pending -= n;
                    __builtin_amdgcn_fence(__ATOMIC_SEQ_CST, "wavefront");
                }
                }
            }
            if (!endsA) next = nextA + takeA;
            else {
                if (lane == 0) { a.b.pathCnt[out][segA] = outCount; a.b.shadowCnt[segA] = shCount; }
                if (takeB) {
                    seg = segB; segBase = baseB; cnt = cntB; next = takeB;
                    outCount = outCountB; shCount = shCountB;
                    haveSeg = true;
                    if (SORT) { permSel ^= 1u; permuted = permutedB; permutedB = false; }
                    if (next >= cnt) {
                        if (lane == 0) { a.b.pathCnt[out][seg] = outCount; a.b.shadowCnt[seg] = shCount; }
                        seg += totalWaves; open_segment();
                    }
                } else if (takeA < 64u) { seg = segB; haveSeg = false; }
                else { seg += totalWaves; open_segment(); }
            }
        }
    }
    block_count_add_uniform<2>(a.counters, { 3, 5 }, { nEntriesOut, nRadiance });
}
template <int MAXL, bool SIMPLE, bool PRIMARY = false>
__global__ __launch_bounds__(kBlock) __attribute__((amdgpu_waves_per_eu(kWavesShade, kWavesShade))) void wf_shade(WfArgs a, HrptPathTracerConstants cb, uint32_t parity, int bounce, int lastBounce)
{
    shade_paths<MAXL, SIMPLE, PRIMARY, false>(a, cb, parity, bounce, lastBounce);
}
template <int MAXL, bool SIMPLE, bool PRIMARY = false>
__global__ __launch_bounds__(kBlock) __attribute__((amdgpu_waves_per_eu(kWavesShade, kWavesShade))) void wf_shade_lt(WfArgs a, HrptPathTracerConstants cb, uint32_t parity, int bounce, int lastBounce)
{
    shade_paths<MAXL, SIMPLE, PRIMARY, true>(a, cb, parity, bounce, lastBounce);
}

template <bool DIRONLY>
__global__ __launch_bounds__(kBlock) void wf_shadow_rays(WfArgs a, HrptPathTracerConstants cb)
{
    const SceneView& s = a.scene;
    const f3 sunDir = mk3(cb.m_SunDirection[0], cb.m_SunDirection[1], cb.m_SunDirection[2]);
    const uint32_t wavesPerBlock = kBlock / 64, lane = lane_id();
    const uint32_t gw = uniform(blockIdx.x * wavesPerBlock + (threadIdx.x >> 6)), totalWaves = gridDim.x * wavesPerBlock;
    for (uint32_t seg = gw; seg < a.numSegments; seg += totalWaves) {
        const uint32_t cnt = uniform(a.b.shadowCnt[seg]), segBase = seg * a.segSize, items = cnt * a.maxLights;
        uint32_t outCount = 0;
        for (uint32_t i0 = 0; i0 < items; i0 += 64) {
            const uint32_t i = i0 + lane;
            bool valid = false; Ray ray; uint32_t id = 0;
            if (i < items) {
                HRT_PHASE(PH_SHADOW_RAYS_ITEM);
                const uint32_t el = i / a.maxLights, j = i - el * a.maxLights, e = segBase + el;
                id = e * a.maxLights + j;
                float4 h4 = a.b.sh4[e];
                if (j < __float_as_uint(h4.w)) {
                    float4 h0 = a.b.sh0[e], h1 = a.b.sh1[e], ls = a.b.shL[(size_t)e * a.maxLights + j];
                    HrptGPULight l = load_light(s, __float_as_uint(ls.z));
                    f3 L; float maxDist;
                    if (nee_direction<DIRONLY>(l, mk3(h1.x, h1.y, h1.z), mk3(h0.x, h0.y, h0.z), sunDir, cb.m_CosSunAngularRadius, ls.x, ls.y, L, maxDist)) {
                        ray = shadow_ray(mk3(h0.x, h0.y, h0.z), L, maxDist);
                        valid = true;
                    }
                }
                if (!valid) a.b.shVis[id] = kVisNoRay;
            }
            const unsigned long long m = __ballot(valid);
            if (valid) {
                const uint32_t o = segBase * a.maxLights + outCount + prefix_rank(m);
                a.b.sqO[o] = make_float4(ray.o.x, ray.o.y, ray.o.z, ray.tmin);
                a.b.sqD[o] = make_float4(ray.d.x, ray.d.y, ray.d.z, ray.tmax);
                a.b.sqId[o] = id;
            }
            outCount += (uint32_t)__popcll(m);
        }
        if (lane == 0) a.b.sqCnt[seg] = outCount;
    }
}

template <bool LDS_BVH, int DEPTH, int W, bool DIRONLY, int MODE, int TL = 0>
__global__ __launch_bounds__(kBlock) __attribute__((amdgpu_waves_per_eu(MODE == 2 && TL == 0 ? 4 : ((MODE == 1 || TL != 0) ? 3 : 1)))) void wf_shadow(WfArgs a, HrptPathTracerConstants cb, int bounce)
{
    static_assert(!TL || (!LDS_BVH && W == 4 && (MODE == kShadowOpaque || MODE == kShadowSlim)), "two-level structure: opaque any-hit query over the global tree");
    static_assert(W != kQuantisedTree || (!LDS_BVH && !TL), "quantised nodes: flat tree in global memory");
    constexpr bool NONOPAQUE = MODE == kShadowBuffered || MODE == kShadowResolve;
    constexpr bool SLIM = MODE == kShadowSlim;
    constexpr int kLdsMax = MODE == kShadowResolve ? kExtendLdsStack : kShadowLdsStack;
    extern __shared__ __attribute__((aligned(128))) char smem[];
    LdsStack<DEPTH, kLdsMax> stack; LdsBvh<W> lbvh;
    constexpr size_t candBytes = MODE == kShadowBuffered ? (size_t)kShadowCandidates * 2 * kBlock * 4 : 0;
    setup_lds<LDS_BVH, DEPTH, W>(smem, a.scene, stack, lbvh, candBytes);
    if (DEPTH > kLdsMax) { stack.spill = a.spill[1] + blockIdx.x * kBlock + threadIdx.x; stack.spillStride = gridDim.x * kBlock; }
    LdsCandidates cand; cand.base = reinterpret_cast<int32_t*>(smem + (size_t)LdsStack<DEPTH, kLdsMax>::kRows * kBlock * 4) + threadIdx.x;
    LdsCandidates3 cand3; cand3.base = cand.base;
    typename GlobalBvhOf<(TL ? kTwoLevelTree : W)>::type gbvh = GlobalBvhOf<(TL ? kTwoLevelTree : W)>::make(a.scene);
    const SceneView& s = a.scene;
    const f3 sunDir = mk3(cb.m_SunDirection[0], cb.m_SunDirection[1], cb.m_SunDirection[2]);
    const float sunIntensity = s.lights[0].m_Intensity;

    const uint32_t wavesPerBlock = kBlock / 64, lane = lane_id();
    const uint32_t gw = uniform(blockIdx.x * wavesPerBlock + (threadIdx.x >> 6)), totalWaves = gridDim.x * wavesPerBlock;
    unsigned int nRays = 0, nSamples = 0, nRadiance = 0, nSkipped16 = 0;
    auto process = [&](uint32_t e) {
                HRT_PHASE(PH_SHADOW_ENTRY);
                if (SLIM) {
                    const float4 h0 = a.b.sh0[e], h1 = a.b.sh1[e];
                    const uint32_t slot = __float_as_uint(h0.w);
                    const float4 rd = a.b.rayD[a.shadowParity][slot];
                    const f3 origin = mk3(h0.x, h0.y, h0.z), N = mk3(h1.x, h1.y, h1.z);
                    uint32_t rng = __float_as_uint(rd.w);
                    const float ux = hrt_rng_next(&rng), uy = hrt_rng_next(&rng);
                    ++nSamples;
                    HrptGPULight l = load_light(s, 0u);
                    f3 L; float maxDist;
                    if (!nee_direction<true>(l, N, origin, sunDir, cb.m_CosSunAngularRadius, ux, uy, L, maxDist)) return;
                    float shadow;
                    if (LDS_BVH) shadow = shadow_query<true>(s, lbvh, origin, L, maxDist, stack);
                    else if constexpr (TL == 2) shadow = shadow_query_two_level_buffered<kTwoLevelCandidates>(s, gbvh, shadow_ray(origin, L, maxDist), stack, cand3);
                    else shadow = shadow_query<true>(s, gbvh, origin, L, maxDist, stack);
                    ++nRays;
                    if (shadow != 0.0f) {
                        const float4 th = a.primary ? make_float4(1.0f, 1.0f, 1.0f, __uint_as_float(slot)) : a.b.thr[a.shadowParity][slot];
                        if (a.primary) ++nSkipped16;
                        const HrptMaterialConstants& mat = s.materials[__float_as_uint(h1.w)];
                        f3 dif, spec;
                        nee_contribution<true>(s, l, nee_lighting(N, mk3(-rd.x, -rd.y, -rd.z), mk3(mat.m_BaseColor), hrt_max(mat.m_RoughnessMetallic[0], 0.04f),
                                                                  mat.m_RoughnessMetallic[1], mat.m_IOR), origin, sunDir, sunIntensity, L, dif, spec);
                        f3 totalDiffuse = mk3(0.0f, 0.0f, 0.0f) + dif * shadow, totalSpecular = mk3(0.0f, 0.0f, 0.0f);
                        if (bounce == 0) totalSpecular = totalSpecular + spec * shadow;
                        const f3 dsum = totalDiffuse + (bounce == 0 ? totalSpecular : mk3(0.0f, 0.0f, 0.0f));
                        if (dsum.x != 0.0f || dsum.y != 0.0f || dsum.z != 0.0f) {
                            const f3 term = mk3(th.x, th.y, th.z) * dsum;
                            const uint32_t smp = __float_as_uint(th.w);
                            float4 r = a.b.radiance[smp];
                            r.x = r.x + term.x; r.y = r.y + term.y; r.z = r.z + term.z;
                            a.b.radiance[smp] = r;
                            ++nRadiance;
                        }
                    }
                    return;
                }
                float4 h0 = a.b.sh0[e], h1 = a.b.sh1[e], h4 = a.b.sh4[e];
                f3 origin = mk3(h0.x, h0.y, h0.z), N = mk3(h1.x, h1.y, h1.z), T = mk3(h4.x, h4.y, h4.z);
                uint32_t smp = __float_as_uint(h0.w), n = __float_as_uint(h4.w);
                nSamples += n;
                f3 totalDiffuse = mk3(0.0f, 0.0f, 0.0f), totalSpecular = mk3(0.0f, 0.0f, 0.0f);
                float4 ls0 = make_float4(0.0f, 0.0f, 0.0f, 0.0f);
                if (MODE != kShadowResolve && n) ls0 = a.b.shL[(size_t)e * a.maxLights];
                for (uint32_t j = 0; j < n; ++j) {
                    HRT_PHASE(PH_SHADOW_SAMPLE);
                    uint32_t vis = kVisCandidates;
                    if (MODE == kShadowResolve) {
                        vis = a.b.shVis[e * a.maxLights + j];
                        if (vis == kVisNoRay) continue;
                        if (vis == kVisBlocked) { ++nRays; continue; }
                    }
                    float4 ls = ls0;
                    if (MODE == kShadowResolve || j) ls = a.b.shL[(size_t)e * a.maxLights + j];
                    HrptGPULight l = load_light(s, __float_as_uint(ls.z));
                    f3 L; float maxDist;
                    if (!nee_direction<DIRONLY>(l, N, origin, sunDir, cb.m_CosSunAngularRadius, ls.x, ls.y, L, maxDist)) continue;
                    float shadow;
                    HRT_PHASE(PH_SHADOW_QUERY);
                    if (MODE == kShadowResolve) {
                        if (vis == kVisClear) shadow = 1.0f;
                        else {
                            Ray sr = shadow_ray(origin, L, maxDist);
                            GlobalCandidates gc; gc.base = a.b.sqCand + (size_t)(e * a.maxLights + j) * kShadowCandidates;
                            const int cnt = (int)((vis >> 8) & 0xFFu); const bool ovf = (vis >> 16) & 1u;
                            if (LDS_BVH) shadow = shadow_resolve_candidates(s, lbvh, sr, make_shear(sr.d), cnt, ovf, gc, stack);
                            else shadow = shadow_resolve_candidates(s, gbvh, sr, make_shear(sr.d), cnt, ovf, gc, stack);
                        }
                    } else if (MODE == kShadowBuffered) {
                        if (LDS_BVH) shadow = shadow_query_buffered<kShadowCandidates>(s, lbvh, origin, L, maxDist, stack, cand);
                        else shadow = shadow_query_buffered<kShadowCandidates>(s, gbvh, origin, L, maxDist, stack, cand);
                    } else {
                        if (LDS_BVH) shadow = shadow_query<true>(s, lbvh, origin, L, maxDist, stack);
                        else if constexpr (TL == 2) shadow = shadow_query_two_level_buffered<kTwoLevelCandidates>(s, gbvh, shadow_ray(origin, L, maxDist), stack, cand3);
                    else shadow = shadow_query<true>(s, gbvh, origin, L, maxDist, stack);
                    }
                    ++nRays;
                    if (shadow != 0.0f) {
                        HRT_PHASE(PH_SHADOW_CONTRIB);
                        float4 h2 = a.b.sh2[e], h3 = a.b.sh3[e];
                        f3 dif, spec;
                        nee_contribution<DIRONLY>(s, l, nee_lighting(N, mk3(h2.x, h2.y, h2.z), mk3(h3.x, h3.y, h3.z), h1.w, h2.w, h3.w), origin, sunDir,
                                                  sunIntensity, L, dif, spec);
                        totalDiffuse = totalDiffuse + dif * shadow;
// ... 69 lines not shown
        accumulation[idx] = acc;
        output[idx] = make_float4(acc.x / acc.w, acc.y / acc.w, acc.z / acc.w, 1.0f);
    }
}

__global__ __launch_bounds__(kBlock) void wf_gbuffer(WfArgs a, HrptPathTracerConstants cb, GBufferPlanes g, uint32_t planeMask)
{
    const uint32_t wavesPerBlock = kBlock / 64, lane = lane_id();
    const uint32_t gw = uniform(blockIdx.x * wavesPerBlock + (threadIdx.x >> 6)), totalWaves = gridDim.x * wavesPerBlock;
    const SceneView& s = a.scene;
    for (uint32_t seg = gw; seg < a.numSegments; seg += totalWaves) {
        const uint32_t cnt = uniform(a.b.pathCnt[0][seg]), segBase = seg * a.segSize;
        for (uint32_t base = 0; base < cnt; base += 64) {
            if (base + lane >= cnt) continue;
            const uint32_t slot = segBase + base + lane;
            const float4 o = a.b.rayO[0][slot], d = a.b.rayD[0][slot], ha = a.b.hit[slot];
            const uint32_t smp = reinterpret_cast<const uint32_t*>(a.b.thr[0] + slot)[3];
            const uint32_t tile = smp >> 6, within = smp & 63u;
            const bool columnMajor = a.rect.stripeCount > 1u;
            const uint32_t den = columnMajor ? a.tilesY : a.tilesX, quo = tile / den, rem = tile - quo * den;
            const uint32_t tcol = columnMajor ? quo : rem, trow = columnMajor ? rem : quo;
            const uint32_t px = a.rect.column_x(tcol) + (within & 7u), py = a.rect.y0 + trow * 8u + (within >> 3);
            uint32_t tri = __float_as_uint(ha.w);
            float4 texel[kGbPlanes];
            if (tri != 0xFFFFFFFFu) {
                tri &= 0x1FFFFFFFu;
                Ray ray; ray.o = mk3(o.x, o.y, o.z); ray.d = mk3(d.x, d.y, d.z); ray.tmin = o.w; ray.tmax = 1e10f;
                Hit h; h.valid = true; h.t = ha.x; h.u = ha.y; h.v = ha.z; h.tri = tri; h.prim = 0; h.inst = s.instances ? a.b.hitInst[slot] : 0u; h.opaque = 1;
                gbuffer_texels(s, cb, ray, h, texel);
            } else gbuffer_miss(texel);
            gbuffer_store(g, planeMask, (size_t)py * a.imageWidth + px, texel);
        }
    }
}

template <bool PLANES>
__global__ __launch_bounds__(kBlock) __attribute__((amdgpu_waves_per_eu(4))) void wf_gbuffer_motion(WfArgs a, HrptPathTracerConstants cb, GBufferPlanes g, uint32_t planeMask, MotionArgs m)
{
    const uint32_t wavesPerBlock = kBlock / 64, lane = lane_id();
    const uint32_t gw = uniform(blockIdx.x * wavesPerBlock + (threadIdx.x >> 6)), totalWaves = gridDim.x * wavesPerBlock;
    const SceneView& s = a.scene;
    for (uint32_t seg = gw; seg < a.numSegments; seg += totalWaves) {
        const uint32_t cnt = uniform(a.b.pathCnt[0][seg]), segBase = seg * a.segSize;
        for (uint32_t base = 0; base < cnt; base += 64) {
            if (base + lane >= cnt) continue;
            const uint32_t slot = segBase + base + lane;
            const float4 o = a.b.rayO[0][slot], d = a.b.rayD[0][slot], ha = a.b.hit[slot];
            const uint32_t smp = reinterpret_cast<const uint32_t*>(a.b.thr[0] + slot)[3];
            const uint32_t tile = smp >> 6, within = smp & 63u;
            const bool columnMajor = a.rect.stripeCount > 1u;
            const uint32_t den = columnMajor ? a.tilesY : a.tilesX, quo = tile / den, rem = tile - quo * den;
            const uint32_t tcol = columnMajor ? quo : rem, trow = columnMajor ? rem : quo;
            const uint32_t px = a.rect.column_x(tcol) + (within & 7u), py = a.rect.y0 + trow * 8u + (within >> 3);
            const size_t idx = (size_t)py * a.imageWidth + px;
            uint32_t tri = __float_as_uint(ha.w);
            float4 texel[kGbPlanes];
            float4 motion = make_float4(0.0f, 0.0f, 0.0f, 0.0f);
            if (tri != 0xFFFFFFFFu) {
                tri &= 0x1FFFFFFFu;
                Hit h; h.valid = true; h.t = ha.x; h.u = ha.y; h.v = ha.z; h.tri = tri; h.prim = 0; h.inst = s.instances ? a.b.hitInst[slot] : 0u; h.opaque = 1;
                const MotionTri mt = motion_gather(s, m, h);
                if constexpr (PLANES) {
                    Ray ray; ray.o = mk3(o.x, o.y, o.z); ray.d = mk3(d.x, d.y, d.z); ray.tmin = o.w; ray.tmax = 1e10f;
                    gbuffer_texels(s, cb, ray, h, texel);
                }
                motion = motion_texel(cb.m_View, m, mt, h.u, h.v);
            } else if constexpr (PLANES) gbuffer_miss(texel);
            if constexpr (PLANES) gbuffer_store(g, planeMask, idx, texel);
            m.plane[idx] = motion;
        }
    }
}

static int resident_blocks_per_cu(const void* kernel, size_t ldsBytes)
{
    static std::mutex mu; static std::unordered_map<uint64_t, int> cache;
    const uint64_t key = (uint64_t)(uintptr_t)kernel * 0x9E3779B97F4A7C15ull ^ (uint64_t)ldsBytes;
    std::lock_guard<std::mutex> lock(mu);
    auto it = cache.find(key);
    if (it != cache.end()) return it->second;
    int n = 0;
    if (hipOccupancyMaxActiveBlocksPerMultiprocessor(&n, kernel, (int)kBlock, ldsBytes) != hipSuccess) { (void)hipGetLastError(); n = 0; }
    cache.emplace(key, n);
    return n;
}
template <class K, class... Args> static void launch_rounds(uint32_t cus, K kernel, dim3 g, size_t ldsBytes, hipStream_t st, Args... args)
{
    const int resident = cus ? resident_blocks_per_cu(reinterpret_cast<const void*>(kernel), ldsBytes) : 0;
    const uint32_t perRound = cus * (uint32_t)(resident > 0 ? resident : 0);
    if (perRound && g.x > perRound) g.x = (g.x / perRound) * perRound;
    hipLaunchKernelGGL(kernel, g, dim3(kBlock), ldsBytes, st, args...);
}

template <int N> using int_c = std::integral_constant<int, N>;
template <class F> void dispatch_variant(const Variant& v, F&& f)
{
    auto depth = [&](auto L, auto W, auto TL) {
        if constexpr (W() == 2) if (v.depth <= 8) return f(L, int_c<8>(), W, TL);
        if (v.depth <= 16) return f(L, int_c<16>(), W, TL);
        if (v.depth <= 32) return f(L, int_c<32>(), W, TL);
        return f(L, int_c<64>(), W, TL);
    };
    if (v.twoLevel) { if (v.twoLevelCandidates) depth(std::false_type(), int_c<4>(), int_c<2>()); else depth(std::false_type(), int_c<4>(), int_c<1>()); }
    else if (v.width == 2) { if (v.lds) depth(std::true_type(), int_c<2>(), int_c<0>()); else depth(std::false_type(), int_c<2>(), int_c<0>()); }
    else if (v.lds) depth(std::true_type(), int_c<4>(), int_c<0>());
    else if (v.quantised) depth(std::false_type(), int_c<kQuantisedTree>(), int_c<0>());
    else depth(std::false_type(), int_c<4>(), int_c<0>());
}

void launch_extend(const Variant& v, uint32_t cus, dim3 g, hipStream_t st, const WfArgs& a, uint32_t parity, bool anyHit = false)
{
    dispatch_variant(v, [&](auto L, auto D, auto W, auto TL) {
        constexpr bool l = L(); constexpr int d = D(), w = W(), tl = TL();
        auto closest = [&](auto kernel) { launch_rounds(cus, kernel, g, v.ldsBytes, st, a, parity); };
        if constexpr (tl != 0) {
            if (a.primary) closest(wf_extend<false, d, 4, false, tl, true>);
            else closest(wf_extend<false, d, 4, false, tl, false>);
        } else if (anyHit) hipLaunchKernelGGL((wf_extend<l, d, w, true>), g, dim3(kBlock), v.ldsBytes + kCandidateLdsBytes, st, a, parity);
        else if constexpr (w == 2) closest(wf_extend<l, d, w, false>);
        else if (a.primary) { if (a.allOpaque) closest(wf_extend<l, d, w, false, 0, true, true>); else closest(wf_extend<l, d, w, false, 0, true>); }
        else { if (a.allOpaque) closest(wf_extend<l, d, w, false, 0, false, true>); else closest(wf_extend<l, d, w, false>); }
    });
}
void launch_shadow(const Variant& v, dim3 g, hipStream_t st, const WfArgs& a, const HrptPathTracerConstants& cb, int bounce, bool dirOnly, int mode)
{
    dispatch_variant(v, [&](auto L, auto D, auto W, auto TL) {
        constexpr bool l = L(); constexpr int d = D(), w = W(), tl = TL();
        auto launch = [&](auto kernel, size_t extraLds) { hipLaunchKernelGGL(kernel, g, dim3(kBlock), v.ldsBytes + extraLds, st, a, cb, bounce); };
        if constexpr (tl != 0) {
            const size_t cand = tl == 2 ? (size_t)kTwoLevelCandidates * 3 * kBlock * 4 : 0;
            if (mode == kShadowSlim) launch(wf_shadow<false, d, 4, true, kShadowSlim, tl>, cand);
            else if (dirOnly) launch(wf_shadow<false, d, 4, true, kShadowOpaque, tl>, cand);
            else launch(wf_shadow<false, d, 4, false, kShadowOpaque, tl>, cand);
        } else if (mode == kShadowResolve) launch(wf_shadow<l, d, w, false, kShadowResolve>, 0);
        else if (mode == kShadowBuffered) launch(wf_shadow<l, d, w, false, kShadowBuffered>, kCandidateLdsBytes);
        else if (mode == kShadowSlim) launch(wf_shadow<l, d, w, true, kShadowSlim>, 0);
        else if (dirOnly) launch(wf_shadow<l, d, w, true, kShadowOpaque>, 0);
        else launch(wf_shadow<l, d, w, false, kShadowOpaque>, 0);
    });
}
void launch_wf_trace_rays(const Variant& v, uint32_t cus, dim3 g, hipStream_t st, const WfTraceArgs& a, bool shadow)
{
    dispatch_variant(v, [&](auto L, auto D, auto W, auto TL) {
        constexpr bool l = L(), tl = TL() != 0; constexpr int d = D(), w = W();
        if constexpr (w != 2) {
            if (shadow) launch_rounds(cus, wf_trace_rays<l, d, w, true, tl>, g, v.ldsBytes + (tl ? 0 : kCandidateLdsBytes), st, a);
            else launch_rounds(cus, wf_trace_rays<l, d, w, false, tl>, g, v.ldsBytes, st, a);
        }
    });
}

TreeCounts tree_counts(const SceneView& scene) { return { scene.nodeCount, scene.node4Count, scene.triCount, scene.nodesQ != nullptr, scene.instances != nullptr, 0u, 0u }; }

}

hipError_t wavefront_trace_rays(WavefrontState& st, const SceneView& scene, const SceneTraits& traits, const HrptRay* rays, HrptRayHit* hits, uint64_t count,
                                bool shadow, hipStream_t stream, std::string& error)
{
    if (count == 0) return hipSuccess;
    hipError_t e; int dev = 0; hipDeviceProp_t prop;
    if ((e = hipGetDevice(&dev)) != hipSuccess || (e = hipGetDeviceProperties(&prop, dev)) != hipSuccess) { error = "hipGetDeviceProperties"; return e; }
    const uint32_t cus = (uint32_t)prop.multiProcessorCount;
    const TraceRaysPlan p = plan_trace_rays(traits, tree_counts(scene), count, shadow, cus, st.knobs);
    WfTraceArgs a{};
    a.scene = scene; a.rays = rays; a.hits = hits; a.count = count;
    a.refillMin = p.refillMin; a.nodeLoopMin = p.nodeLoopMin; a.quantised = p.v.quantised;
    if (p.spillEntries) {
        const size_t bytes = p.spillThreads * p.spillEntries * 4;
        if (bytes > st.traceSpillBytes) {
            if (st.traceSpill) { (void)hipStreamSynchronize(stream); (void)hipFree(st.traceSpill); st.traceSpill = nullptr; st.traceSpillBytes = 0; }
            if ((e = hipMalloc(&st.traceSpill, bytes)) != hipSuccess) { error = "hipMalloc(traversal stack overflow)"; return e; }
            st.traceSpillBytes = bytes;
        }
        a.spill = static_cast<int32_t*>(st.traceSpill);
    }
    launch_wf_trace_rays(p.v, cus, dim3(p.grid), stream, a, shadow);
    if ((e = hipGetLastError()) != hipSuccess) { error = "kernel launch"; return e; }
    return hipSuccess;
}

bool wavefront_supports(const SceneView& scene, const HrptPathTracerConstants& cb)
{
    (void)scene;
    return cb.m_MaxBounces >= 1;
}

void wavefront_release(WavefrontState& st)
{
    if (st.pool) (void)hipFree(st.pool);
    st.pool = nullptr; st.poolBytes = 0;
    if (st.spill) (void)hipFree(st.spill);
    st.spill = nullptr; st.spillBytes = 0;
    if (st.traceSpill) (void)hipFree(st.traceSpill);
    st.traceSpill = nullptr; st.traceSpillBytes = 0;
    if (st.gbPool) (void)hipFree(st.gbPool);
    st.gbPool = nullptr; st.gbPoolBytes = 0;
    for (hipEvent_t e : st.events) (void)hipEventDestroy(e);
    st.events.clear(); st.eventsUsed = 0;
    for (hipEvent_t e : st.forkEvents) (void)hipEventDestroy(e);
    for (hipEvent_t e : st.joinEvents) (void)hipEventDestroy(e);
    st.forkEvents.clear(); st.joinEvents.clear();
    if (st.auxStream) (void)hipStreamDestroy(st.auxStream);
    st.auxStream = nullptr;
}

void wavefront_collect_timing(WavefrontState& st)
{
    for (uint32_t i = 0; i + 1 < st.eventsUsed; i += 2) {
        float t = 0.0f;
        if (hipEventElapsedTime(&t, st.events[i], st.events[i + 1]) == hipSuccess) { st.kernelMs[st.kind[i / 2]] += t; st.kernelLaunches[st.kind[i / 2]]++; }
    }
    st.eventsUsed = 0;
}

#ifdef HRPT_SKY_DEBUG
extern "C" int hrpt_sky_debug_read(float* out) { return hipMemcpyFromSymbol(out, HIP_SYMBOL(g_skyDebug), sizeof(float) * 2048 * 16) == hipSuccess ? 0 : -3; }
#endif
#ifdef HRPT_PHASE_PROFILE
extern "C" int hrpt_phase_profile_read(unsigned long long* out128)
{
    if (hipMemcpyFromSymbol(out128, HIP_SYMBOL(g_phaseCounters), 128 * sizeof(unsigned long long)) != hipSuccess) return -3;
    static const unsigned long long zero[128] = { 0 };
    if (hipMemcpyToSymbol(HIP_SYMBOL(g_phaseCounters), zero, sizeof zero) != hipSuccess) return -3;
    return 0;
}
#endif

void wavefront_reset_timing(WavefrontState& st)
{
    st.eventsUsed = 0;
    for (int k = 0; k < 5; ++k) { st.kernelMs[k] = 0.0f; st.kernelLaunches[k] = 0; }
    st.raygenBytes = 0; st.resolveBytes = 0;
}

void wavefront_queue_bytes(const WavefrontState& st, const DeviceCounters& c, uint64_t& trace, uint64_t& shade, uint64_t& shadow)
{
    const uint64_t path = st.plan.pathRecordBytes, survivors = c.closestRays > c.paths ? c.closestRays - c.paths : 0;
    trace = c.closestRays * (32 + 16);
    shade = c.closestRays * (path + 16) + survivors * path + c.neeEntries * 80 + c.neeSamples * 16 + c.radianceShade * 32;
    shadow = c.neeEntries * 48 + c.neeSamples * 16 + c.radianceShadow * (32 + 32);
    if (st.plan.shadowMode == kShadowSlim) {
        shade = c.closestRays * (path + 16) + survivors * path + c.neeEntries * 32 + c.radianceShade * 32;
        shadow = c.neeEntries * (32 + 16) + c.radianceShadow * (16 + 32);
    }
    if (st.plan.shadowMode == kShadowResolve) shadow += c.neeEntries * 32 + c.neeSamples * 16 + c.shadowRays * 72 + c.neeEntries * st.plan.maxLights * 8;
    if (st.plan.fusedPrimary) {
        trace -= c.paths * 16;
        shade = shade - c.paths * (path - 16) + c.paths * 16;
        shadow -= c.skipped16 * 16;
    }
}

namespace {
bool timing_mark(WavefrontState& st, hipStream_t stream, int kind, bool begin)
{
    if (st.eventsUsed >= 4096) return true;
    if (st.eventsUsed + 1 > st.events.size()) {
        hipEvent_t e;
        if (hipEventCreate(&e) != hipSuccess) return false;
        st.events.push_back(e);
    }
    if (begin) { if (st.kind.size() < st.eventsUsed / 2 + 1) st.kind.resize(st.eventsUsed / 2 + 1); st.kind[st.eventsUsed / 2] = (uint8_t)kind; }
    (void)hipEventRecord(st.events[st.eventsUsed], stream);
    st.eventsUsed++;
    return true;
}

size_t carve_pool(char* base, WfArgs& a, uint64_t capacity, uint32_t segs, uint32_t maxLights, const SceneTraits& traits, bool hasInstances)
{
    const bool hasMedium = traits.hasMedium, hasShadowRayQueue = traits.hasNonOpaque || maxLights > 1;
    size_t off = 0;
    auto carve = [&](auto*& stream, size_t bytes, bool present = true) {
        stream = reinterpret_cast<std::remove_reference_t<decltype(stream)>>(reinterpret_cast<uintptr_t>(base) + (present ? off : 0));
        if (present) off += (bytes + 255) & ~(size_t)255;
    };
    WfBuffers& b = a.b;
    for (int p = 0; p < 2; ++p) {
        carve(b.rayO[p], capacity * 16); carve(b.rayD[p], capacity * 16); carve(b.thr[p], capacity * 16);
        carve(b.med0[p], capacity * 16, hasMedium); carve(b.med1[p], capacity * 16, hasMedium);
        carve(b.pathCnt[p], (size_t)segs * 4);
    }
    carve(b.hit, capacity * 16);
    carve(b.hitInst, capacity * 4, hasInstances); if (!hasInstances) b.hitInst = nullptr;
    carve(a.primaryArgs, sizeof(PrimaryArgs));
    carve(b.sh0, capacity * 16); carve(b.sh1, capacity * 16); carve(b.sh2, capacity * 16); carve(b.sh3, capacity * 16); carve(b.sh4, capacity * 16);
    carve(b.shL, capacity * 16 * maxLights);
    carve(b.shadowCnt, (size_t)segs * 4); carve(b.radiance, capacity * 16);
    carve(b.sqO, capacity * 16 * maxLights, hasShadowRayQueue); carve(b.sqD, capacity * 16 * maxLights, hasShadowRayQueue); carve(b.sqId, capacity * 4 * maxLights, hasShadowRayQueue);
    carve(b.sqCnt, (size_t)segs * 4, hasShadowRayQueue); carve(b.shVis, capacity * 4 * maxLights, hasShadowRayQueue); carve(b.sqCand, capacity * 8 * kShadowCandidates * maxLights, hasShadowRayQueue);
    return off;
}
}

hipError_t wavefront_render(WavefrontState& st, const SceneView& scene, const SceneTraits& traits, const HrptPathTracerConstants& constants,
                            uint32_t accumCount, float4* accumulation, float4* output, uint32_t width, uint32_t height, TileRect rect,
                            DeviceCounters* counters, hipStream_t stream, std::string& error)
{
    (void)height;
    if (rect.x1 <= rect.x0 || rect.y1 <= rect.y0 || rect.columns() == 0) return hipSuccess;
    hipError_t e;
    int dev = 0; hipDeviceProp_t prop;
    if ((e = hipGetDevice(&dev)) != hipSuccess || (e = hipGetDeviceProperties(&prop, dev)) != hipSuccess) { error = "hipGetDeviceProperties"; return e; }
    const uint32_t cus = (uint32_t)prop.multiProcessorCount;
    TreeCounts tree = tree_counts(scene);
    tree.instanceCount = st.shadeInstances; tree.materialCount = st.shadeMaterials;
    const RenderPlan& plan = st.plan = plan_render(traits, tree, constants.m_LightCount, cus, st.knobs);
    const uint32_t maxLights = plan.maxLights;
    const uint32_t tilesX = rect.columns(), tilesY = (rect.y1 - rect.y0 + 7) / 8;
    const uint64_t pixelsPadded = (uint64_t)tilesX * tilesY * 64;
    uint32_t sppPerBatch = accumCount < kMaxSppPerBatch ? accumCount : kMaxSppPerBatch;
    uint64_t maxSamples = 64ull << 20;
    if (pixelsPadded * sppPerBatch * plan.bytesPerSample > st.poolBytes) {
        size_t freeB = 0, totalB = 0;
        if (hipMemGetInfo(&freeB, &totalB) == hipSuccess) {
            const uint64_t budget = (uint64_t)(freeB + st.poolBytes) / 2;
            if (budget / plan.bytesPerSample < maxSamples) maxSamples = budget / plan.bytesPerSample;
        }
    }
    if (maxSamples * maxLights > 0xFFFFFFFFull) maxSamples = 0xFFFFFFFFull / maxLights;
    while (sppPerBatch > 1 && pixelsPadded * sppPerBatch > maxSamples) --sppPerBatch;
    WfArgs a{};
    uint64_t capacity = 0; uint32_t segs = 0;
    for (;;) {
        capacity = ((pixelsPadded * sppPerBatch + kMaxSegment - 1) / kMaxSegment) * kMaxSegment;
        if (capacity >= (1ull << 31)) { error = "tile too large for one batch"; return hipErrorInvalidValue; }
        segs = (uint32_t)(capacity / 64);
        const size_t bytes = carve_pool(nullptr, a, capacity, segs, maxLights, traits, scene.instances != nullptr);
        if (bytes <= st.poolBytes) break;
        if (st.pool) { (void)hipStreamSynchronize(stream); if (st.auxStream) (void)hipStreamSynchronize(st.auxStream); (void)hipFree(st.pool); st.pool = nullptr; st.poolBytes = 0; }
        e = hipMalloc(&st.pool, bytes);
        if (e == hipSuccess) { st.poolBytes = bytes; break; }
        (void)hipGetLastError();
        if (sppPerBatch == 1) {
            error = "hipMalloc(queue pool, " + std::to_string(bytes >> 20) + " MiB for " + std::to_string(capacity) + " samples; render a smaller tile)";
            return e;
        }
        sppPerBatch = (sppPerBatch + 1) / 2;
    }
    carve_pool(static_cast<char*>(st.pool), a, capacity, segs, maxLights, traits, scene.instances != nullptr);
    if (plan.spillEntries) {
        const size_t bytes = 2 * plan.spillThreads * plan.spillEntries * 4;
        if (bytes > st.spillBytes) {
            if (st.spill) { (void)hipStreamSynchronize(stream); if (st.auxStream) (void)hipStreamSynchronize(st.auxStream); (void)hipFree(st.spill); st.spill = nullptr; st.spillBytes = 0; }
            if ((e = hipMalloc(&st.spill, bytes)) != hipSuccess) { error = "hipMalloc(traversal stack overflow)"; return e; }
            st.spillBytes = bytes;
        }
        a.spill[0] = static_cast<int32_t*>(st.spill); a.spill[1] = a.spill[0] + plan.spillThreads * plan.spillEntries;
    }
    a.scene = scene;
    a.tilesX = tilesX; a.tilesY = tilesY; a.rect = rect; a.imageWidth = width; a.pixelsPadded = (uint32_t)pixelsPadded;
    a.maxLights = maxLights; a.hasMedium = traits.hasMedium ? 1u : 0u; a.hasStochasticAlpha = traits.hasStochasticAlpha ? 1u : 0u; a.allOpaque = traits.hasNonOpaque ? 0u : 1u;
    a.counters = counters;
    a.refillMin = st.knobs.refillMin ? st.knobs.refillMin : kRefillMinDefault; a.streamSegments = st.knobs.drainSegments ? 0u : 1u; a.sortShade = plan.sortShade; a.nodeLoopMin = plan.nodeLoopMin;
    a.slimShadow = plan.slim ? 1u : 0u;
    a.shadeInstances = tree.instanceCount; a.shadeMaterials = tree.materialCount;
    const bool fusedPrimary = plan.fusedPrimary;

    for (uint32_t first = 0; first < accumCount; first += sppPerBatch) {
        const uint32_t spp = (accumCount - first) < sppPerBatch ? (accumCount - first) : sppPerBatch;
        a.spp = spp; a.numSamples = (uint32_t)(pixelsPadded * spp);
        const BatchPlan batch = plan_batch(plan, st.knobs, a.numSamples);
        a.segSize = batch.segSize; a.numSegments = batch.numSegments;
        const dim3 grid(batch.grid);

        HrptPathTracerConstants cb = constants;
        cb.m_AccumulationIndex = constants.m_AccumulationIndex + first;
        JitterTable jt;
        for (uint32_t k = 0; k < spp; ++k) {
            jt.j[k].x = hrpt_halton(cb.m_AccumulationIndex + k + 1, 2) - 0.5f;
            jt.j[k].y = hrpt_halton(cb.m_AccumulationIndex + k + 1, 3) - 0.5f;
        }
        PrimaryArgs pr{};
        if (fusedPrimary) {
            for (int i = 0; i < 16; ++i) pr.clipToWorld[i] = cb.m_View.m_MatClipToWorldNoOffset[i];
            for (int i = 0; i < 3; ++i) pr.cam[i] = cb.m_CameraPos[i];
            pr.invW = cb.m_View.m_ViewportSizeInv[0]; pr.invH = cb.m_View.m_ViewportSizeInv[1]; pr.accumIndex = cb.m_AccumulationIndex;
            for (uint32_t k = 0; k < spp; ++k) pr.j[k] = jt.j[k];
            hipLaunchKernelGGL(wf_store_primary, dim3(1), dim3(64), 0, stream, pr, const_cast<PrimaryArgs*>(a.primaryArgs));
        }
        const bool timedEnds = st.profile && st.eventsUsed + 4 <= 4096;
        if (!fusedPrimary) {
            if (timedEnds) timing_mark(st, stream, 3, true);
            hipLaunchKernelGGL(wf_raygen, grid, dim3(kBlock), 0, stream, a, cb, jt);
            if (timedEnds) timing_mark(st, stream, 3, false);
        }
        {
            const uint64_t w = (uint64_t)rect.columns() * 8u, px = (w < rect.x1 - rect.x0 ? w : (uint64_t)rect.x1 - rect.x0) * (rect.y1 - rect.y0);
            if (!fusedPrimary) st.raygenBytes += (uint64_t)a.numSamples * 16 + px * spp * st.plan.pathRecordBytes;
            st.resolveBytes += px * ((uint64_t)spp * 16 + 32 + (cb.m_AccumulationIndex > 0 ? 16 : 0));
        }
        const int maxBounces = (int)cb.m_MaxBounces;
        bool overlap = !st.profile && !st.knobs.serialShadow && maxBounces > 1;
        if (overlap) {
            if (!st.auxStream && hipStreamCreateWithFlags(&st.auxStream, hipStreamNonBlocking) != hipSuccess) { st.auxStream = nullptr; overlap = false; }
            while (overlap && st.forkEvents.size() < (size_t)maxBounces) {
                hipEvent_t f, j;
                if (hipEventCreateWithFlags(&f, hipEventDisableTiming) != hipSuccess) { overlap = false; break; }
                if (hipEventCreateWithFlags(&j, hipEventDisableTiming) != hipSuccess) { (void)hipEventDestroy(f); overlap = false; break; }
                st.forkEvents.push_back(f); st.joinEvents.push_back(j);
            }
        }
        auto shadow_stage = [&](hipStream_t sst, int bounce) {
            a.shadowParity = (uint32_t)bounce & 1u;
            if (plan.shadowMode == kShadowResolve) {
                if (traits.directionalLightsOnly) hipLaunchKernelGGL((wf_shadow_rays<true>), grid, dim3(kBlock), 0, sst, a, cb);
                else hipLaunchKernelGGL((wf_shadow_rays<false>), grid, dim3(kBlock), 0, sst, a, cb);
                launch_extend(plan.vA, cus, grid, sst, a, 0u, true);
            }
            launch_shadow(plan.vS, grid, sst, a, cb, bounce, traits.directionalLightsOnly, plan.shadowMode);
        };
        bool pendingJoin = false;
        for (int bounce = 0; bounce < maxBounces; ++bounce) {
            const uint32_t parity = (uint32_t)bounce & 1u;
            const bool timed = st.profile && st.eventsUsed + 8 <= 4096;
            if (timed) timing_mark(st, stream, 0, true);
            a.primary = (fusedPrimary && bounce == 0) ? 1u : 0u;
            launch_extend(plan.vE, cus, dim3(batch.gridExtend), stream, a, parity);
            if (timed) { timing_mark(st, stream, 0, false); timing_mark(st, stream, 1, true); }
            if (pendingJoin) { if ((e = hipStreamWaitEvent(stream, st.joinEvents[(size_t)bounce - 1], 0)) != hipSuccess) { error = "hipStreamWaitEvent(join)"; return e; } pendingJoin = false; }
            const int last = bounce + 1 == maxBounces ? 1 : 0;
            const size_t sortLds = (size_t)(kBlock / 64) * ((size_t)5 * a.segSize);
            if (maxLights > kMaxLights) hipLaunchKernelGGL((wf_shade<0, false>), grid, dim3(kBlock), sortLds, stream, a, cb, parity, bounce, last);
            else if (maxLights > 1) hipLaunchKernelGGL((wf_shade<(int)kMaxLights, false>), grid, dim3(kBlock), sortLds, stream, a, cb, parity, bounce, last);
            else if (plan.simpleScene && plan.shadeLdsTables && a.primary) hipLaunchKernelGGL((wf_shade_lt<1, true, true>), grid, dim3(kBlock), plan.shadeLdsBytes, stream, a, cb, parity, bounce, last);
            else if (plan.simpleScene && plan.shadeLdsTables) hipLaunchKernelGGL((wf_shade_lt<1, true>), grid, dim3(kBlock), plan.shadeLdsBytes, stream, a, cb, parity, bounce, last);
            else if (plan.simpleScene && a.primary) hipLaunchKernelGGL((wf_shade<1, true, true>), grid, dim3(kBlock), plan.shadeLdsBytes, stream, a, cb, parity, bounce, last);
            else if (plan.simpleScene) hipLaunchKernelGGL((wf_shade<1, true>), grid, dim3(kBlock), plan.shadeLdsBytes, stream, a, cb, parity, bounce, last);
            else hipLaunchKernelGGL((wf_shade<1, false>), grid, dim3(kBlock), sortLds, stream, a, cb, parity, bounce, last);
            if (timed) { timing_mark(st, stream, 1, false); timing_mark(st, stream, 2, true); }
            if (overlap) {
                if ((e = hipEventRecord(st.forkEvents[(size_t)bounce], stream)) != hipSuccess ||
                    (e = hipStreamWaitEvent(st.auxStream, st.forkEvents[(size_t)bounce], 0)) != hipSuccess) { error = "fork to the shadow stream"; return e; }
                shadow_stage(st.auxStream, bounce);
                if ((e = hipEventRecord(st.joinEvents[(size_t)bounce], st.auxStream)) != hipSuccess) { error = "hipEventRecord(join)"; return e; }
                pendingJoin = true;
            } else {
                shadow_stage(stream, bounce);
            }
            if (timed) timing_mark(st, stream, 2, false);
        }
        if (pendingJoin && (e = hipStreamWaitEvent(stream, st.joinEvents[(size_t)maxBounces - 1], 0)) != hipSuccess) { error = "hipStreamWaitEvent(join)"; return e; }
        uint32_t rgrid = (uint32_t)((pixelsPadded + kBlock - 1) / kBlock); if (rgrid > cus * 8) rgrid = cus * 8;
        if (timedEnds) timing_mark(st, stream, 4, true);
        hipLaunchKernelGGL(wf_resolve, dim3(rgrid), dim3(kBlock), 0, stream, a, accumulation, output, cb.m_AccumulationIndex);
        if (timedEnds) timing_mark(st, stream, 4, false);
        if ((e = hipGetLastError()) != hipSuccess) { error = "kernel launch"; return e; }
    }
    return hipSuccess;
}

namespace {
size_t carve_gbuffer_pool(char* base, WfArgs& a, uint64_t capacity, uint32_t segs, bool hasMedium, bool hasInstances)
{
    size_t off = 0;
    auto carve = [&](auto*& stream, size_t bytes, bool present = true) {
        stream = reinterpret_cast<std::remove_reference_t<decltype(stream)>>(reinterpret_cast<uintptr_t>(base) + (present ? off : 0));
        if (present) off += (bytes + 255) & ~(size_t)255;
    };
    WfBuffers& b = a.b;
    carve(b.rayO[0], capacity * 16); carve(b.rayD[0], capacity * 16); carve(b.thr[0], capacity * 16);
    carve(b.med0[0], capacity * 16, hasMedium); carve(b.med1[0], capacity * 16, hasMedium);
    carve(b.pathCnt[0], (size_t)segs * 4);
    carve(b.hit, capacity * 16);
    carve(b.hitInst, capacity * 4, hasInstances); if (!hasInstances) b.hitInst = nullptr;
    carve(b.radiance, capacity * 16);
    carve(a.counters, sizeof(DeviceCounters) * kCounterShards);
    return off;
}
}

hipError_t wavefront_gbuffer(WavefrontState& st, const SceneView& scene, const SceneTraits& traits, const HrptPathTracerConstants& constants,
                             float4* const* planes, uint32_t planeMask, uint32_t width, TileRect rect, hipStream_t stream, std::string& error, const MotionArgs* motion)
{
    if (rect.x1 <= rect.x0 || rect.y1 <= rect.y0 || rect.columns() == 0) return hipSuccess;
    hipError_t e;
    int dev = 0; hipDeviceProp_t prop;
    if ((e = hipGetDevice(&dev)) != hipSuccess || (e = hipGetDeviceProperties(&prop, dev)) != hipSuccess) { error = "hipGetDeviceProperties"; return e; }
    const uint32_t cus = (uint32_t)prop.multiProcessorCount;
    const uint32_t tilesX = rect.columns(), tilesY = (rect.y1 - rect.y0 + 7) / 8;
    const uint64_t pixelsPadded = (uint64_t)tilesX * tilesY * 64;
    const uint64_t capacity = ((pixelsPadded + kMaxSegment - 1) / kMaxSegment) * kMaxSegment;
    if (capacity >= (1ull << 31)) { error = "tile too large for one batch"; return hipErrorInvalidValue; }
    const GBufferPlan plan = plan_gbuffer(traits, tree_counts(scene), cus, st.knobs, (uint32_t)pixelsPadded);
    WfArgs a{};
    const uint32_t segs = (uint32_t)(capacity / 64);
    const size_t bytes = carve_gbuffer_pool(nullptr, a, capacity, segs, traits.hasMedium, scene.instances != nullptr);
    char* pool = static_cast<char*>(st.pool);
    if (bytes > st.poolBytes) {
        if (bytes > st.gbPoolBytes) {
            if (st.gbPool) { (void)hipStreamSynchronize(stream); (void)hipFree(st.gbPool); st.gbPool = nullptr; st.gbPoolBytes = 0; }
            if ((e = hipMalloc(&st.gbPool, bytes)) != hipSuccess) { error = "hipMalloc(G-buffer queue pool, " + std::to_string(bytes >> 20) + " MiB)"; return e; }
            st.gbPoolBytes = bytes;
        }
        pool = static_cast<char*>(st.gbPool);
    }
    carve_gbuffer_pool(pool, a, capacity, segs, traits.hasMedium, scene.instances != nullptr);
    if (plan.spillEntries) {
        const size_t spillBytes = 2 * plan.spillThreads * plan.spillEntries * 4;
        if (spillBytes > st.spillBytes) {
            if (st.spill) { (void)hipStreamSynchronize(stream); if (st.auxStream) (void)hipStreamSynchronize(st.auxStream); (void)hipFree(st.spill); st.spill = nullptr; st.spillBytes = 0; }
            if ((e = hipMalloc(&st.spill, spillBytes)) != hipSuccess) { error = "hipMalloc(traversal stack overflow)"; return e; }
            st.spillBytes = spillBytes;
        }
        a.spill[0] = static_cast<int32_t*>(st.spill); a.spill[1] = a.spill[0] + plan.spillThreads * plan.spillEntries;
    }
    a.scene = scene;
    a.tilesX = tilesX; a.tilesY = tilesY; a.rect = rect; a.imageWidth = width; a.pixelsPadded = (uint32_t)pixelsPadded;
    a.spp = 1; a.numSamples = (uint32_t)pixelsPadded; a.segSize = plan.batch.segSize; a.numSegments = plan.batch.numSegments;
    a.maxLights = 1; a.hasMedium = traits.hasMedium ? 1u : 0u; a.hasStochasticAlpha = traits.hasStochasticAlpha ? 1u : 0u; a.allOpaque = traits.hasNonOpaque ? 0u : 1u;
    a.refillMin = st.knobs.refillMin ? st.knobs.refillMin : kRefillMinDefault; a.streamSegments = st.knobs.drainSegments ? 0u : 1u; a.nodeLoopMin = plan.nodeLoopMin;
    a.primary = 0u;
    JitterTable jt{};
    jt.j[0].x = constants.m_Jitter[0]; jt.j[0].y = constants.m_Jitter[1];
    GBufferPlanes g; for (uint32_t k = 0; k < kGbPlanes; ++k) g.plane[k] = planes[k];
    const dim3 grid(plan.batch.grid);
    hipLaunchKernelGGL(wf_raygen, grid, dim3(kBlock), 0, stream, a, constants, jt);
    launch_extend(plan.vE, cus, dim3(plan.batch.gridExtend), stream, a, 0u);
    if (motion && planeMask != 0u) hipLaunchKernelGGL(wf_gbuffer_motion<true>, grid, dim3(kBlock), 0, stream, a, constants, g, planeMask, *motion);
    else if (motion) hipLaunchKernelGGL(wf_gbuffer_motion<false>, grid, dim3(kBlock), 0, stream, a, constants, g, planeMask, *motion);
    else hipLaunchKernelGGL(wf_gbuffer, grid, dim3(kBlock), 0, stream, a, constants, g, planeMask);
    if ((e = hipGetLastError()) != hipSuccess) { error = "kernel launch"; return e; }
    return hipSuccess;
}

}
```

hobbyrenderer_amd/csrc/pt_wavefront_plan.h:

```cpp
#pragma once

#include <stddef.h>
#include <stdint.h>

namespace hrt {

struct SceneTraits {
    bool hasMedium = false;
    bool hasStochasticAlpha = false;
    bool hasTextures = false;
    bool hasTransmissiveOrBlend = false;
    bool directionalLightsOnly = true;
    bool hasNonOpaque = false;
    uint32_t bvhMaxDepth = 0;
    uint32_t bvh4MaxDepth = 0;
    bool quantisedNodes = false;
    uint32_t twoLevelStackNeed = 0;
};

struct TreeCounts {
    uint32_t nodeCount = 0, node4Count = 0, triCount = 0;
    bool hasNodesQ = false, hasInstances = false;
    uint32_t instanceCount = 0, materialCount = 0;
};

struct WavefrontKnobs {
    uint32_t blocksPerCu = 0;
    uint32_t extendBlocksPerCu = 0;
    uint32_t refillMin = 0;
    uint32_t segmentShift = 0;
    uint32_t segmentSize = 0;
    bool drainSegments = false;
    bool serialShadow = false;
    uint32_t padLdsBytes = 0;
    uint32_t bvhWidth = 0;
    uint32_t nodeLoopMin = ~0u;
    bool noFusedPrimary = false;
    bool noSlimShadow = false;
    int shadeSort = -1;
    bool noShadeLdsTables = false;
    int shadowPath = 0;
};

constexpr uint32_t kMaxSegment = 1024;
constexpr uint32_t kBlock = 256;
constexpr uint32_t kMaxLights = 8;
constexpr size_t kLdsBudget = 64 * 1024;
constexpr int kExtendLdsStack = 16, kShadowLdsStack = 32;
constexpr uint32_t kMaxStackNeed = 128;
constexpr int kShadowCandidates = 8;
constexpr int kTwoLevelCandidates = 4;
constexpr size_t kCandidateLdsBytes = (size_t)kShadowCandidates * 2 * kBlock * 4;
#ifndef HRPT_LDS_NODE4_STRIDE
#define HRPT_LDS_NODE4_STRIDE 128
#endif
constexpr uint32_t kLdsNode4Stride = HRPT_LDS_NODE4_STRIDE;
static_assert(kLdsNode4Stride >= 128 && kLdsNode4Stride % 32 == 0, "LDS node stride: 128 bytes of node, near / far rows 32-byte aligned");
constexpr uint32_t kRefillMinDefault = 12;
constexpr uint32_t kShadeRing = 64, kShadeRingFields = 23;
constexpr size_t kShadeRingBytes = (size_t)(kBlock / 64) * kShadeRing * kShadeRingFields * 4;
constexpr uint32_t kShadeBlocksPerCu = 4;
constexpr size_t kCuLdsBytes = 160 * 1024, kShadeLdsMargin = 1024;
constexpr size_t kShadeLdsPerBlock = kCuLdsBytes / kShadeBlocksPerCu - kShadeLdsMargin;
constexpr size_t kTriAttrBytes = 80, kInstShadeBytes = 48, kMaterialBytes = 180;
inline size_t shade_table_bytes(uint32_t triCount, uint32_t instanceCount, uint32_t materialCount)
{
    const size_t b = (size_t)triCount * kTriAttrBytes + (size_t)instanceCount * kInstShadeBytes + (size_t)materialCount * kMaterialBytes;
    return (b + 15) & ~(size_t)15;
}
enum : int { kShadowOpaque = 0, kShadowBuffered = 1, kShadowResolve = 2, kShadowSlim = 3 };

struct Variant { bool lds = false; int depth = 0, width = 0; size_t ldsBytes = 0; bool twoLevel = false; bool twoLevelCandidates = false; bool quantised = false; };

inline uint32_t stack_entries4(uint32_t depth4) { return 3 * depth4 + 3; }
inline uint32_t stack_need4(const SceneTraits& traits) { return traits.twoLevelStackNeed ? traits.twoLevelStackNeed : stack_entries4(traits.bvh4MaxDepth); }

inline Variant pick_variant(const SceneTraits& traits, const TreeCounts& tree, int width, size_t extraBytes, int ldsStackMax, size_t padBytes)
{
    Variant v; v.width = width;
    uint32_t need = traits.twoLevelStackNeed;
    if (need) { v.width = 4; v.twoLevel = true; v.twoLevelCandidates = traits.hasNonOpaque; }
    else {
        if (v.width == 4 && stack_entries4(traits.bvh4MaxDepth) > kMaxStackNeed) v.width = 2;
        need = v.width == 2 ? traits.bvhMaxDepth + 2 : stack_entries4(traits.bvh4MaxDepth);
    }
    v.depth = (v.width == 2 && need <= 8) ? 8 : (need <= 16 ? 16 : (need <= 32 ? 32 : 64));
    const size_t bvhBytes = v.twoLevel ? 0 : (v.width == 2 ? (size_t)tree.nodeCount * 64 : (size_t)tree.node4Count * kLdsNode4Stride) + (size_t)tree.triCount * 48;
    const size_t stackBytes = (size_t)(v.depth > ldsStackMax ? ldsStackMax : v.depth) * kBlock * 4;
    v.lds = bvhBytes > 0 && stackBytes + extraBytes + bvhBytes <= kLdsBudget;
    v.ldsBytes = stackBytes + (v.lds ? bvhBytes : 0) + padBytes;
    v.quantised = v.width == 4 && !v.lds && !v.twoLevel && traits.quantisedNodes && tree.hasNodesQ;
    return v;
}

struct RenderPlan {
    Variant vE, vS, vA;
    int shadowMode = kShadowOpaque;
    bool slim = false;
    bool simpleScene = false;
    bool fusedPrimary = false;
    uint32_t sortShade = 0, nodeLoopMin = 0;
    uint32_t maxLights = 1, cus = 0, blocksPerCu = 0, extendBlocksPerCu = 0;
    uint32_t spillEntries = 0; size_t spillThreads = 0;
    uint32_t pathRecordBytes = 48; uint64_t bytesPerSample = 0;
    bool shadeLdsTables = false;
    size_t shadeTableBytes = 0;
    size_t shadeLdsBytes = 0;
};
struct BatchPlan { uint32_t segSize, numSegments, grid, gridExtend; };

inline RenderPlan plan_render(const SceneTraits& traits, const TreeCounts& tree, uint32_t lightCount, uint32_t cus, const WavefrontKnobs& k)
{
    RenderPlan p;
    const uint32_t maxLights = lightCount ? lightCount : 1;
    p.maxLights = maxLights; p.cus = cus;
    p.bytesPerSample = 16ull * (2 * (3 + (traits.hasMedium ? 2 : 0)) + 1 + 5 + maxLights + 1) + (tree.hasInstances ? 4 : 0) +
                       ((traits.hasNonOpaque || maxLights > 1) ? (16ull + 16 + 4 + 4 + 8 * kShadowCandidates) * maxLights : 0);
    p.pathRecordBytes = traits.hasMedium ? 80u : 48u;
    p.sortShade = k.shadeSort < 0 ? (traits.hasTextures ? 1u : 0u) : (uint32_t)k.shadeSort;
    const size_t candBytes = traits.hasNonOpaque ? kCandidateLdsBytes : 0;
    auto pick = [&](int width, size_t extraBytes, int ldsStackMax) { return pick_variant(traits, tree, width, extraBytes, ldsStackMax, k.padLdsBytes); };
    const int forced = k.bvhWidth == 2 ? 2 : (k.bvhWidth == 4 ? 4 : 0);
    p.vE = pick(forced ? forced : 4, 0, kExtendLdsStack);
    p.vS = pick(forced ? forced : 4, candBytes, kShadowLdsStack);
    if (!forced && p.vS.lds && !traits.hasNonOpaque) p.vS = pick(2, candBytes, kShadowLdsStack);
    const bool manyLights = maxLights > 1;
    const bool unevenRays = manyLights || (traits.hasNonOpaque && traits.hasTransmissiveOrBlend);
    const int selfMode = traits.hasNonOpaque ? kShadowBuffered : kShadowOpaque;
    p.shadowMode = (!p.vS.lds && unevenRays) ? kShadowResolve : selfMode;
    if (k.shadowPath == 1) p.shadowMode = selfMode;
    if (k.shadowPath == 2 && (traits.hasNonOpaque || manyLights)) p.shadowMode = kShadowResolve;
    if (traits.twoLevelStackNeed) p.shadowMode = kShadowOpaque;
    p.vA = pick(forced ? forced : 4, kCandidateLdsBytes, kExtendLdsStack);
    if (p.shadowMode == kShadowResolve) p.vS = pick(forced ? forced : 4, 0, kExtendLdsStack);
    p.simpleScene = !traits.hasTextures && !traits.hasTransmissiveOrBlend && traits.directionalLightsOnly;
    p.slim = p.simpleScene && !manyLights && p.shadowMode == kShadowOpaque && !k.noSlimShadow;
    if (p.slim) p.shadowMode = kShadowSlim;
    p.nodeLoopMin = k.nodeLoopMin != ~0u ? k.nodeLoopMin : (p.vE.lds ? 16u : 24u);
    p.blocksPerCu = k.blocksPerCu ? k.blocksPerCu : ((k.serialShadow && !p.vE.lds) ? 8 : 16);
    p.extendBlocksPerCu = k.extendBlocksPerCu ? k.extendBlocksPerCu : (k.blocksPerCu ? k.blocksPerCu : (p.vE.lds ? 12u : 6u));
    if (p.vE.depth > kExtendLdsStack || p.vS.depth > kShadowLdsStack) {
        const uint32_t worst = traits.twoLevelStackNeed ? traits.twoLevelStackNeed : (p.vE.width == 4 || p.vS.width == 4 ? stack_entries4(traits.bvh4MaxDepth) : traits.bvhMaxDepth + 2);
        p.spillEntries = worst > (uint32_t)kExtendLdsStack ? worst - kExtendLdsStack : 1u;
        p.spillThreads = (size_t)cus * (p.blocksPerCu > p.extendBlocksPerCu ? p.blocksPerCu : p.extendBlocksPerCu) * kBlock;
    }
    p.shadeLdsBytes = kShadeRingBytes;
    if (p.simpleScene && !manyLights && !k.noShadeLdsTables && !tree.hasInstances && !traits.twoLevelStackNeed &&
        tree.triCount && tree.instanceCount && tree.materialCount) {
        const size_t tables = shade_table_bytes(tree.triCount, tree.instanceCount, tree.materialCount);
        if (kShadeRingBytes + tables <= kShadeLdsPerBlock) { p.shadeLdsTables = true; p.shadeTableBytes = tables; p.shadeLdsBytes = kShadeRingBytes + tables; }
    }
    p.fusedPrimary = p.simpleScene && !manyLights && maxLights <= kMaxLights && p.vE.width == 4 && !traits.hasMedium && !traits.hasStochasticAlpha && !k.noFusedPrimary;
    return p;
}

inline BatchPlan plan_batch(const RenderPlan& p, const WavefrontKnobs& k, uint32_t numSamples)
{
    BatchPlan b;
    const bool largeBatch = numSamples >= (8u << 20) && p.maxLights == 1 && p.vE.lds;
    uint32_t shift = k.segmentShift ? k.segmentShift : (largeBatch ? 9u : 8u);
    if (shift < 6) shift = 6;
    if (shift > 10) shift = 10;
    b.segSize = 1u << shift;
    if (k.segmentSize >= 64u && k.segmentSize <= kMaxSegment) b.segSize = k.segmentSize;
    b.numSegments = (numSamples + b.segSize - 1) / b.segSize;
    const uint32_t wavesNeeded = b.numSegments, blocksNeeded = (wavesNeeded + 3) / 4;
    b.grid = p.cus * p.blocksPerCu; if (b.grid > blocksNeeded) b.grid = blocksNeeded; if (b.grid == 0) b.grid = 1;
    b.gridExtend = p.cus * p.extendBlocksPerCu; if (b.gridExtend > blocksNeeded) b.gridExtend = blocksNeeded; if (b.gridExtend == 0) b.gridExtend = 1;
    return b;
}

struct GBufferPlan {
    Variant vE; BatchPlan batch;
    uint32_t nodeLoopMin = 0, pathRecordBytes = 48;
    uint32_t spillEntries = 0; size_t spillThreads = 0;
    uint64_t bytesPerSample = 0;
};
inline GBufferPlan plan_gbuffer(const SceneTraits& traits, const TreeCounts& tree, uint32_t cus, const WavefrontKnobs& k, uint32_t numSamples)
{
    const RenderPlan p = plan_render(traits, tree, 1, cus, k);
    GBufferPlan g;
    g.vE = p.vE; g.batch = plan_batch(p, k, numSamples);
    g.nodeLoopMin = p.nodeLoopMin; g.pathRecordBytes = p.pathRecordBytes;
    g.spillEntries = p.spillEntries; g.spillThreads = p.spillThreads;
    g.bytesPerSample = p.pathRecordBytes + 16u + (tree.hasInstances ? 4u : 0u) + 16u;
    return g;
}

struct TraceRaysPlan {
    Variant v;
    uint32_t grid = 0, refillMin = 0, nodeLoopMin = 0;
    uint32_t spillEntries = 0; size_t spillThreads = 0;
};
inline bool wavefront_trace_rays_supported(const SceneTraits& traits) { return stack_need4(traits) <= kMaxStackNeed; }
inline TraceRaysPlan plan_trace_rays(const SceneTraits& traits, const TreeCounts& tree, uint64_t count, bool shadow, uint32_t cus, const WavefrontKnobs& k)
{
    TraceRaysPlan p;
    p.v = pick_variant(traits, tree, 4, shadow ? kCandidateLdsBytes : 0, kExtendLdsStack, 0);
    const uint32_t blocksPerCu = k.blocksPerCu ? k.blocksPerCu : 16;
    const uint64_t chunks = (count + 255) / 256, blocksNeeded = (chunks + 3) / 4;
    p.grid = cus * blocksPerCu; if (p.grid > blocksNeeded) p.grid = (uint32_t)blocksNeeded;
    p.refillMin = k.refillMin ? k.refillMin : kRefillMinDefault;
    p.nodeLoopMin = k.nodeLoopMin != ~0u ? k.nodeLoopMin : (p.v.lds ? 16u : 24u);
    if (p.v.depth > kExtendLdsStack) {
        const uint32_t need = stack_need4(traits);
        p.spillEntries = need > (uint32_t)kExtendLdsStack ? need - kExtendLdsStack : 1u;
        p.spillThreads = (size_t)cus * blocksPerCu * kBlock;
    }
    return p;
}

}
```

Baseline: 26400 Mrays/s.

## Fuse bounce-0 extend and shade into one wf_bounce0 kernel for simple scenes

For simple single-light scenes with LDS tables and an LDS-resident 4-wide BVH, bounce 0 now runs a fused kernel that traces primary rays and shades them in the same pass. This drops the separate extend launch and the hit and ray write and read round-trip through global memory. The shade body is factored into a reusable shade_iteration with a configurable ring size, which uses a smaller 32-entry ring to make room for the tree copy in LDS. The cost is higher LDS use per block and more register pressure, which can lower occupancy. Device CU count is also cached instead of queried on every call.

Measured after the change: 27710 Mrays/s, median of 6. 1.05x the previous value.

```diff
diff --git a/hobbyrenderer_amd/csrc/pt_capi.cpp b/hobbyrenderer_amd/csrc/pt_capi.cpp
--- a/hobbyrenderer_amd/csrc/pt_capi.cpp
+++ b/hobbyrenderer_amd/csrc/pt_capi.cpp
@@ -182,6 +182,7 @@
     if (const char* e = getenv("HRPT_WF_SHADE_SORT")) c->wf.knobs.shadeSort = atoi(e) != 0 ? 1 : 0;
     if (const char* e = getenv("HRPT_WF_SLIM_SHADOW")) c->wf.knobs.noSlimShadow = atoi(e) == 0;
     if (const char* e = getenv("HRPT_WF_FUSED_PRIMARY")) c->wf.knobs.noFusedPrimary = atoi(e) == 0;
+    if (const char* e = getenv("HRPT_WF_FUSED_BOUNCE0")) c->wf.knobs.noFusedBounce0 = atoi(e) == 0;
     if (const char* e = getenv("HRPT_WF_SHADE_LDS_TABLES")) c->wf.knobs.noShadeLdsTables = atoi(e) == 0;
     if (const char* e = getenv("HRPT_WF_NODE_LOOP_MIN")) c->wf.knobs.nodeLoopMin = (uint32_t)atoi(e);
     if (const char* e = getenv("HRPT_BLOOM_FUSED_TAIL")) { const int v = atoi(e); c->bloomTailTexels = v == 1 ? 8192u : (v > 0 ? (uint32_t)v : 0u); }
@@ -1112,6 +1113,7 @@
     for (int i = 0; i < kCounterShards; ++i) {
         total.closestRays += h[i].closestRays; total.shadowRays += h[i].shadowRays; total.paths += h[i].paths; total.neeEntries += h[i].neeEntries;
         total.neeSamples += h[i].neeSamples; total.radianceShade += h[i].radianceShade; total.radianceShadow += h[i].radianceShadow; total.skipped16 += h[i].skipped16;
+        total.fusedPaths += h[i].fusedPaths; total.fusedEntries += h[i].fusedEntries;
     }
     out->closestRays = total.closestRays; out->shadowRays = total.shadowRays; out->paths = total.paths;
     out->neeEntries = total.neeEntries; out->neeSamples = total.neeSamples;
diff --git a/hobbyrenderer_amd/csrc/pt_kernels.h b/hobbyrenderer_amd/csrc/pt_kernels.h
--- a/hobbyrenderer_amd/csrc/pt_kernels.h
+++ b/hobbyrenderer_amd/csrc/pt_kernels.h
@@ -21,6 +21,8 @@
     unsigned long long radianceShade;
     unsigned long long radianceShadow;
     unsigned long long skipped16;
+    unsigned long long fusedPaths;
+    unsigned long long fusedEntries;
 };
 
 struct TileRect {
diff --git a/hobbyrenderer_amd/csrc/pt_wavefront.h b/hobbyrenderer_amd/csrc/pt_wavefront.h
--- a/hobbyrenderer_amd/csrc/pt_wavefront.h
+++ b/hobbyrenderer_amd/csrc/pt_wavefront.h
@@ -32,6 +32,7 @@
     RenderPlan plan;
     uint32_t shadeInstances = 0, shadeMaterials = 0;
     WavefrontKnobs knobs;
+    uint32_t cus = 0;
     bool profile = false;
     hipStream_t auxStream = nullptr;
     std::vector<hipEvent_t> forkEvents, joinEvents;
diff --git a/hobbyrenderer_amd/csrc/pt_wavefront.hip b/hobbyrenderer_amd/csrc/pt_wavefront.hip
--- a/hobbyrenderer_amd/csrc/pt_wavefront.hip
+++ b/hobbyrenderer_amd/csrc/pt_wavefront.hip
@@ -633,90 +633,21 @@
 }
 
 
-template <int MAXL, bool SIMPLE, bool PRIMARY, bool LDS_TABLES>
-HRT_DEV void shade_paths(const WfArgs& a, const HrptPathTracerConstants& cb, uint32_t parity, int bounce, int lastBounce)
-{
-    static_assert(!PRIMARY || SIMPLE, "no raygen pass: SIMPLE scenes only");
-    static_assert(!LDS_TABLES || SIMPLE, "tables in LDS: behind the ring of the SIMPLE variants");
-    const uint32_t wavesPerBlock = kBlock / 64, lane = lane_id();
-    const uint32_t gw = uniform(blockIdx.x * wavesPerBlock + (threadIdx.x >> 6)), totalWaves = gridDim.x * wavesPerBlock;
-    const uint32_t in = parity, out = parity ^ 1u;
+struct ShadeLane { bool valid, inA; uint32_t slot; float4 o, d, t, ha; };
+struct ShadeWave { uint32_t outCount = 0, shCount = 0, ringHead = 0, pending = 0; unsigned int nEntriesOut = 0, nRadiance = 0; };
+template <int MAXL, bool SIMPLE, bool PRIMARY, uint32_t RING, bool FUSED, class TABLES>
+HRT_DEV void shade_iteration(const WfArgs& a, const HrptPathTracerConstants& cb, const TABLES& tables, float* const ring, uint32_t in, uint32_t out, int bounce, int lastBounce,
+                             const ShadeLane& L, uint32_t baseA, uint32_t baseB, bool endsA, ShadeWave& w, uint32_t& outCountB, uint32_t& shCountB)
+{
+    static_assert(!FUSED || (PRIMARY && SIMPLE && MAXL == 1), "wf_bounce0: the bounce-0 SIMPLE single-light body");
+    static_assert((RING & (RING - 1u)) == 0u && RING >= 1u && RING <= 64u, "ring positions are masked; one flush takes at most 64 entries");
+    constexpr uint32_t kRing = RING;
     const SceneView& s = a.scene;
-    extern __shared__ __attribute__((aligned(16))) char shadeSmem[];
-    constexpr uint32_t kRing = kShadeRing, kRingFields = kShadeRingFields;
-    float* const ring = reinterpret_cast<float*>(shadeSmem) + (size_t)uniform(threadIdx.x >> 6) * kRing * kRingFields;
-    LdsShadeTables ldsTables; ldsTables.attrs = ldsTables.instShade = ldsTables.materials = 0u;
-    if constexpr (LDS_TABLES) { ldsTables = copy_shade_tables(shadeSmem + kShadeRingBytes, a); __syncthreads(); }
-    const GlobalShadeTables globalTables{ s };
-    auto shade_hit = [&](PathState& ps, const Hit& h, SurfaceCarry& carry, auto&& emit) {
-        if constexpr (LDS_TABLES) return shade_surface_a<!SIMPLE, !SIMPLE, SIMPLE>(s, ldsTables, cb, ps, h, carry, emit);
-        else return shade_surface_a<!SIMPLE, !SIMPLE, SIMPLE>(s, globalTables, cb, ps, h, carry, emit);
-    };
-    uint32_t ringHead = 0, pending = 0;
-    unsigned int nEntriesOut = 0, nRadiance = 0;
-    constexpr bool SORT = !SIMPLE;
-    const uint32_t segSize = a.segSize;
-    uint16_t* const permBase = reinterpret_cast<uint16_t*>(shadeSmem) + (size_t)uniform(threadIdx.x >> 6) * segSize * 2;
-    uint8_t* const keys = reinterpret_cast<uint8_t*>(shadeSmem) + (size_t)wavesPerBlock * segSize * 4 + (size_t)uniform(threadIdx.x >> 6) * segSize;
-    uint32_t permSel = 0;
-    bool permuted = false, permutedB = false;
-    auto sort_segment = [&](uint32_t base, uint32_t n, uint16_t* perm) -> bool {
-        HRT_PHASE(PH_SHADE_SORT);
-        uint32_t c0 = 0, c1 = 0, c2 = 0;
-        for (uint32_t b = 0; b < n; b += 64) {
-            const uint32_t e = b + lane; uint32_t k = 4u;
-            if (e < n) { k = __float_as_uint(a.b.hit[base + e].w) >> 29; k = k > 3u ? 3u : k; keys[e] = (uint8_t)k; }
-            c0 += (uint32_t)__popcll(__ballot(k == 0u)); c1 += (uint32_t)__popcll(__ballot(k == 1u)); c2 += (uint32_t)__popcll(__ballot(k == 2u));
-        }
-        const uint32_t c3 = n - c0 - c1 - c2;
-        if (c0 == n || c1 == n || c2 == n || c3 == n) return false;
-        __builtin_amdgcn_fence(__ATOMIC_SEQ_CST, "wavefront");
-        uint32_t b0 = 0, b1 = c0, b2 = c0 + c1, b3 = c0 + c1 + c2;
-        for (uint32_t b = 0; b < n; b += 64) {
-            const uint32_t e = b + lane; const uint32_t k = e < n ? keys[e] : 4u;
-            const unsigned long long m0 = __ballot(k == 0u), m1 = __ballot(k == 1u), m2 = __ballot(k == 2u), m3 = __ballot(k == 3u);
-            if (k == 0u) perm[b0 + prefix_rank(m0)] = (uint16_t)e;
-            if (k == 1u) perm[b1 + prefix_rank(m1)] = (uint16_t)e;
-            if (k == 2u) perm[b2 + prefix_rank(m2)] = (uint16_t)e;
-            if (k == 3u) perm[b3 + prefix_rank(m3)] = (uint16_t)e;
-            b0 += (uint32_t)__popcll(m0); b1 += (uint32_t)__popcll(m1); b2 += (uint32_t)__popcll(m2); b3 += (uint32_t)__popcll(m3);
-        }
-        __builtin_amdgcn_fence(__ATOMIC_SEQ_CST, "wavefront");
-        return true;
-    };
-    {
-        uint32_t seg = gw, cnt = 0, segBase = 0, next = 0, outCount = 0, shCount = 0;
-        bool haveSeg = false;
-        auto open_segment = [&]() {
-            haveSeg = false; cnt = 0; next = 0; outCount = 0; shCount = 0;
-            for (; seg < a.numSegments; seg += totalWaves) {
-                cnt = uniform(PRIMARY ? path_count(a, in, seg) : a.b.pathCnt[in][seg]);
-                if (cnt) { segBase = seg * a.segSize; haveSeg = true; break; }
-                if (lane == 0) { a.b.pathCnt[out][seg] = 0; a.b.shadowCnt[seg] = 0; }
-            }
-            if (SORT && a.sortShade && haveSeg) permuted = sort_segment(segBase, cnt, permBase + permSel * segSize);
-        };
-        open_segment();
-        while (haveSeg) {
-            const uint32_t takeA = cnt - next < 64u ? cnt - next : 64u;
-            const uint32_t segA = seg, baseA = segBase, nextA = next;
-            const bool endsA = nextA + takeA >= cnt;
-            uint32_t takeB = 0, segB = 0, baseB = 0, cntB = 0;
-            if (endsA && takeA < 64u) {
-                uint32_t probe = seg + totalWaves;
-                for (; probe < a.numSegments; probe += totalWaves) {
-                    cntB = uniform(PRIMARY ? path_count(a, in, probe) : a.b.pathCnt[in][probe]);
-                    if (cntB) break;
-                    if (lane == 0) { a.b.pathCnt[out][probe] = 0; a.b.shadowCnt[probe] = 0; }
-                }
-                if (probe < a.numSegments) {
-                    segB = probe; baseB = probe * a.segSize; takeB = cntB < 64u - takeA ? cntB : 64u - takeA;
-                    if (SORT && a.sortShade) permutedB = sort_segment(baseB, cntB, permBase + (permSel ^ 1u) * segSize);
-                } else segB = probe;
-            }
-            const bool inA = lane < takeA;
-            uint32_t outCountB = 0, shCountB = 0;
-            bool valid = lane < takeA + takeB, alive = false, wantDefer = false, wantRadiance = false;
+    const uint32_t lane = lane_id();
+    const bool inA = L.inA;
+    uint32_t& outCount = w.outCount; uint32_t& shCount = w.shCount;
+    outCountB = 0; shCountB = 0;
+            bool valid = L.valid, alive = false, wantDefer = false, wantRadiance = false;
             LobeDraw ld; ld.spec = false; ld.specProb = 0.0f; ld.root = 0.0f; ld.sp = 0.0f; ld.cp = 0.0f;
             uint32_t nNee = 0, smp = 0, slotIn = 0;
             PathState ps; f3 neeT = mk3(0.0f, 0.0f, 0.0f);
@@ -724,16 +655,10 @@
             NeeBuf<(STREAMED ? 1 : MAXL)> nee; SurfaceCarry carry;
             if (valid) {
                 HRT_PHASE(PH_SHADE_ITER);
-                uint32_t slot = inA ? baseA + ((SORT && permuted) ? (uint32_t)permBase[permSel * segSize + nextA + lane] : nextA + lane)
-                                    : baseB + ((SORT && permutedB) ? (uint32_t)permBase[(permSel ^ 1u) * segSize + (lane - takeA)] : lane - takeA);
+                const uint32_t slot = L.slot;
                 slotIn = slot;
-                float4 o, d, t;
-                if constexpr (PRIMARY) {
-                    const PrimaryArgs& pr = *a.primaryArgs;
-                    o = make_float4(pr.cam[0], pr.cam[1], pr.cam[2], 0.0f); d = a.b.rayD[in][slot];
-                    t = make_float4(1.0f, 1.0f, 1.0f, __uint_as_float(slot));
-                } else { o = a.b.rayO[in][slot]; d = a.b.rayD[in][slot]; t = a.b.thr[in][slot]; }
-                float4 ha = a.b.hit[slot]; uint32_t tri = __float_as_uint(ha.w);
+                const float4 o = L.o, d = L.d, t = L.t, ha = L.ha;
+                uint32_t tri = __float_as_uint(ha.w);
                 const bool noPath = PRIMARY && tri == kNoPathRecord;
                 if (tri < kNoPathRecord) tri &= 0x1FFFFFFFu;
                 ps.ray.o = mk3(o.x, o.y, o.z); ps.ray.d = mk3(d.x, d.y, d.z); ps.ray.tmin = o.w; ps.ray.tmax = 1e10f;
@@ -750,7 +675,7 @@
                     HRT_PHASE(PH_SHADE_HIT);
                     Hit h; h.valid = true; h.t = ha.x; h.u = ha.y; h.v = ha.z; h.tri = tri; h.prim = 0; h.inst = s.instances ? a.b.hitInst[slot] : 0u; h.opaque = 1;
                     f3 emissiveTerm = mk3(0.0f, 0.0f, 0.0f);
-                    SurfaceOutcome oc = shade_hit(ps, h, carry, [&](uint32_t li, float ux, float uy) {
+                    SurfaceOutcome oc = shade_surface_a<!SIMPLE, !SIMPLE, SIMPLE>(s, tables, cb, ps, h, carry, [&](uint32_t li, float ux, float uy) {
                         if (STREAMED) ++nNee;
                         else if (nNee < (uint32_t)MAXL) { nee.ux[nNee] = ux; nee.uy[nNee] = uy; nee.light[nNee] = li; ++nNee; }
                     });
@@ -790,7 +715,7 @@
                 if (lastBounce) alive = false;
                 wantRadiance = addRadiance && !PRIMARY;
             }
-            nRadiance += (unsigned int)__popcll(__ballot(wantRadiance));
+            w.nRadiance += (unsigned int)__popcll(__ballot(wantRadiance));
             const unsigned long long mA = __ballot(alive && inA), mB = __ballot(alive && !inA);
             if (alive) {
                 HRT_PHASE(PH_SHADE_WRITE);
@@ -808,6 +733,7 @@
                 uint32_t e = inA ? baseA + shCount + prefix_rank(msA) : baseB + prefix_rank(msB);
                 a.b.sh0[e] = make_float4(carry.worldPos.x, carry.worldPos.y, carry.worldPos.z, __uint_as_float(slotIn));
                 a.b.sh1[e] = make_float4(carry.N.x, carry.N.y, carry.N.z, __uint_as_float(carry.material));
+                if constexpr (FUSED) a.b.rayD[in][slotIn] = L.d;
             } else if (nNee > 0) {
                 uint32_t e = inA ? baseA + shCount + prefix_rank(msA) : baseB + prefix_rank(msB);
                 a.b.sh0[e] = make_float4(carry.worldPos.x, carry.worldPos.y, carry.worldPos.z, __uint_as_float(smp));
@@ -831,15 +757,19 @@
             }
             outCount += (uint32_t)__popcll(mA); shCount += (uint32_t)__popcll(msA);
             outCountB = (uint32_t)__popcll(mB); shCountB = (uint32_t)__popcll(msB);
-            nEntriesOut += (unsigned int)(__popcll(msA) + __popcll(msB));
+            w.nEntriesOut += (unsigned int)(__popcll(msA) + __popcll(msB));
             if (SIMPLE) {
                 const unsigned long long md = __ballot(wantDefer);
                 const uint32_t nNew = (uint32_t)__popcll(md);
+                uint32_t first = 0;
                 bool parked = false;
-                for (int round = 0; round < 2 && !parked; ++round) {
-                parked = pending + nNew <= kRing;
-                if (parked && wantDefer) {
-                    float* e = ring + ((ringHead + pending + prefix_rank(md)) & (kRing - 1u));
+                for (int round = 0; round < (kRing < 64u ? 3 : 2) && !parked; ++round) {
+                uint32_t nPark = nNew - first;
+                if (w.pending + nPark <= kRing) parked = true;
+                else nPark = (kRing < 64u && w.pending == 0u) ? kRing : 0u;
+                const uint32_t rank = prefix_rank(md) - first;
+                if (wantDefer && (kRing < 64u ? rank < nPark : parked)) {
+                    float* e = ring + ((w.ringHead + w.pending + rank) & (kRing - 1u));
                     e[0 * kRing] = carry.N.x; e[1 * kRing] = carry.N.y; e[2 * kRing] = carry.N.z;
                     e[3 * kRing] = carry.V.x; e[4 * kRing] = carry.V.y; e[5 * kRing] = carry.V.z;
                     e[6 * kRing] = carry.F0.x; e[7 * kRing] = carry.F0.y; e[8 * kRing] = carry.F0.z;
@@ -848,13 +778,13 @@
                     e[17 * kRing] = ps.throughput.x; e[18 * kRing] = ps.throughput.y; e[19 * kRing] = ps.throughput.z;
                     e[20 * kRing] = __uint_as_float(ps.rng); e[21 * kRing] = __uint_as_float(smp); e[22 * kRing] = inA ? 1.0f : 0.0f;
                 }
-                if (parked) pending += nNew;
+                w.pending += nPark; first += nPark;
                 __builtin_amdgcn_fence(__ATOMIC_SEQ_CST, "wavefront");
-                while (pending >= 64u || ((endsA || !parked) && pending)) {
-                    const uint32_t n = pending < 64u ? pending : 64u;
+                while (w.pending >= 64u || ((endsA || !parked) && w.pending)) {
+                    const uint32_t n = w.pending < 64u ? w.pending : 64u;
                     bool alive2 = false, tagA = true; PathState q; uint32_t smp2 = 0;
                     if (lane < n) {
-                        const float* e = ring + ((ringHead + lane) & (kRing - 1u));
+                        const float* e = ring + ((w.ringHead + lane) & (kRing - 1u));
                         f3 N = mk3(e[0 * kRing], e[1 * kRing], e[2 * kRing]), V = mk3(e[3 * kRing], e[4 * kRing], e[5 * kRing]), F0 = mk3(e[6 * kRing], e[7 * kRing], e[8 * kRing]);
                         LobeDraw d2; d2.spec = true; d2.root = e[10 * kRing]; d2.sp = e[11 * kRing]; d2.cp = e[12 * kRing]; d2.specProb = e[13 * kRing];
                         f3 wp = mk3(e[14 * kRing], e[15 * kRing], e[16 * kRing]);
@@ -870,11 +800,105 @@
                         a.b.thr[out][o] = make_float4(q.throughput.x, q.throughput.y, q.throughput.z, __uint_as_float(smp2));
                     }
                     outCount += (uint32_t)__popcll(m2A); outCountB += (uint32_t)__popcll(m2B);
-                    ringHead = (ringHead + n) & (kRing - 1u); pending -= n;
+                    w.ringHead = (w.ringHead + n) & (kRing - 1u); w.pending -= n;
                     __builtin_amdgcn_fence(__ATOMIC_SEQ_CST, "wavefront");
                 }
                 }
             }
+}
+
+template <int MAXL, bool SIMPLE, bool PRIMARY, bool LDS_TABLES>
+HRT_DEV void shade_paths(const WfArgs& a, const HrptPathTracerConstants& cb, uint32_t parity, int bounce, int lastBounce)
+{
+    static_assert(!PRIMARY || SIMPLE, "no raygen pass: SIMPLE scenes only");
+    static_assert(!LDS_TABLES || SIMPLE, "tables in LDS: behind the ring of the SIMPLE variants");
+    const uint32_t wavesPerBlock = kBlock / 64, lane = lane_id();
+    const uint32_t gw = uniform(blockIdx.x * wavesPerBlock + (threadIdx.x >> 6)), totalWaves = gridDim.x * wavesPerBlock;
+    const uint32_t in = parity, out = parity ^ 1u;
+    const SceneView& s = a.scene;
+    extern __shared__ __attribute__((aligned(16))) char shadeSmem[];
+    constexpr uint32_t kRing = kShadeRing, kRingFields = kShadeRingFields;
+    float* const ring = reinterpret_cast<float*>(shadeSmem) + (size_t)uniform(threadIdx.x >> 6) * kRing * kRingFields;
+    LdsShadeTables ldsTables; ldsTables.attrs = ldsTables.instShade = ldsTables.materials = 0u;
+    if constexpr (LDS_TABLES) { ldsTables = copy_shade_tables(shadeSmem + kShadeRingBytes, a); __syncthreads(); }
+    const GlobalShadeTables globalTables{ s };
+    ShadeWave w;
+    uint32_t& outCount = w.outCount; uint32_t& shCount = w.shCount;
+    constexpr bool SORT = !SIMPLE;
+    const uint32_t segSize = a.segSize;
+    uint16_t* const permBase = reinterpret_cast<uint16_t*>(shadeSmem) + (size_t)uniform(threadIdx.x >> 6) * segSize * 2;
+    uint8_t* const keys = reinterpret_cast<uint8_t*>(shadeSmem) + (size_t)wavesPerBlock * segSize * 4 + (size_t)uniform(threadIdx.x >> 6) * segSize;
+    uint32_t permSel = 0;
+    bool permuted = false, permutedB = false;
+    auto sort_segment = [&](uint32_t base, uint32_t n, uint16_t* perm) -> bool {
+        HRT_PHASE(PH_SHADE_SORT);
+        uint32_t c0 = 0, c1 = 0, c2 = 0;
+        for (uint32_t b = 0; b < n; b += 64) {
+            const uint32_t e = b + lane; uint32_t k = 4u;
+            if (e < n) { k = __float_as_uint(a.b.hit[base + e].w) >> 29; k = k > 3u ? 3u : k; keys[e] = (uint8_t)k; }
+            c0 += (uint32_t)__popcll(__ballot(k == 0u)); c1 += (uint32_t)__popcll(__ballot(k == 1u)); c2 += (uint32_t)__popcll(__ballot(k == 2u));
+        }
+        const uint32_t c3 = n - c0 - c1 - c2;
+        if (c0 == n || c1 == n || c2 == n || c3 == n) return false;
+        __builtin_amdgcn_fence(__ATOMIC_SEQ_CST, "wavefront");
+        uint32_t b0 = 0, b1 = c0, b2 = c0 + c1, b3 = c0 + c1 + c2;
+        for (uint32_t b = 0; b < n; b += 64) {
+            const uint32_t e = b + lane; const uint32_t k = e < n ? keys[e] : 4u;
+            const unsigned long long m0 = __ballot(k == 0u), m1 = __ballot(k == 1u), m2 = __ballot(k == 2u), m3 = __ballot(k == 3u);
+            if (k == 0u) perm[b0 + prefix_rank(m0)] = (uint16_t)e;
+            if (k == 1u) perm[b1 + prefix_rank(m1)] = (uint16_t)e;
+            if (k == 2u) perm[b2 + prefix_rank(m2)] = (uint16_t)e;
+            if (k == 3u) perm[b3 + prefix_rank(m3)] = (uint16_t)e;
+            b0 += (uint32_t)__popcll(m0); b1 += (uint32_t)__popcll(m1); b2 += (uint32_t)__popcll(m2); b3 += (uint32_t)__popcll(m3);
+        }
+        __builtin_amdgcn_fence(__ATOMIC_SEQ_CST, "wavefront");
+        return true;
+    };
+    {
+        uint32_t seg = gw, cnt = 0, segBase = 0, next = 0;
+        bool haveSeg = false;
+        auto open_segment = [&]() {
+            haveSeg = false; cnt = 0; next = 0; outCount = 0; shCount = 0;
+            for (; seg < a.numSegments; seg += totalWaves) {
+                cnt = uniform(PRIMARY ? path_count(a, in, seg) : a.b.pathCnt[in][seg]);
+                if (cnt) { segBase = seg * a.segSize; haveSeg = true; break; }
+                if (lane == 0) { a.b.pathCnt[out][seg] = 0; a.b.shadowCnt[seg] = 0; }
+            }
+            if (SORT && a.sortShade && haveSeg) permuted = sort_segment(segBase, cnt, permBase + permSel * segSize);
+        };
+        open_segment();
+        while (haveSeg) {
+            const uint32_t takeA = cnt - next < 64u ? cnt - next : 64u;
+            const uint32_t segA = seg, baseA = segBase, nextA = next;
+            const bool endsA = nextA + takeA >= cnt;
+            uint32_t takeB = 0, segB = 0, baseB = 0, cntB = 0;
+            if (endsA && takeA < 64u) {
+                uint32_t probe = seg + totalWaves;
+                for (; probe < a.numSegments; probe += totalWaves) {
+                    cntB = uniform(PRIMARY ? path_count(a, in, probe) : a.b.pathCnt[in][probe]);
+                    if (cntB) break;
+                    if (lane == 0) { a.b.pathCnt[out][probe] = 0; a.b.shadowCnt[probe] = 0; }
+                }
+                if (probe < a.numSegments) {
+                    segB = probe; baseB = probe * a.segSize; takeB = cntB < 64u - takeA ? cntB : 64u - takeA;
+                    if (SORT && a.sortShade) permutedB = sort_segment(baseB, cntB, permBase + (permSel ^ 1u) * segSize);
+                } else segB = probe;
+            }
+            ShadeLane L; L.valid = lane < takeA + takeB; L.inA = lane < takeA; L.slot = 0;
+            if (L.valid) {
+                const uint32_t slot = L.inA ? baseA + ((SORT && permuted) ? (uint32_t)permBase[permSel * segSize + nextA + lane] : nextA + lane)
+                                          : baseB + ((SORT && permutedB) ? (uint32_t)permBase[(permSel ^ 1u) * segSize + (lane - takeA)] : lane - takeA);
+                L.slot = slot;
+                if constexpr (PRIMARY) {
+                    const PrimaryArgs& pr = *a.primaryArgs;
+                    L.o = make_float4(pr.cam[0], pr.cam[1], pr.cam[2], 0.0f); L.d = a.b.rayD[in][slot];
+                    L.t = make_float4(1.0f, 1.0f, 1.0f, __uint_as_float(slot));
+                } else { L.o = a.b.rayO[in][slot]; L.d = a.b.rayD[in][slot]; L.t = a.b.thr[in][slot]; }
+                L.ha = a.b.hit[slot];
+            }
+            uint32_t outCountB = 0, shCountB = 0;
+            if constexpr (LDS_TABLES) shade_iteration<MAXL, SIMPLE, PRIMARY, kShadeRing, false>(a, cb, ldsTables, ring, in, out, bounce, lastBounce, L, baseA, baseB, endsA, w, outCountB, shCountB);
+            else shade_iteration<MAXL, SIMPLE, PRIMARY, kShadeRing, false>(a, cb, globalTables, ring, in, out, bounce, lastBounce, L, baseA, baseB, endsA, w, outCountB, shCountB);
             if (!endsA) next = nextA + takeA;
             else {
                 if (lane == 0) { a.b.pathCnt[out][segA] = outCount; a.b.shadowCnt[segA] = shCount; }
@@ -892,7 +916,7 @@
             }
         }
     }
-    block_count_add_uniform<2>(a.counters, { 3, 5 }, { nEntriesOut, nRadiance });
+    block_count_add_uniform<2>(a.counters, { 3, 5 }, { w.nEntriesOut, w.nRadiance });
 }
 template <int MAXL, bool SIMPLE, bool PRIMARY = false>
 __global__ __launch_bounds__(kBlock) __attribute__((amdgpu_waves_per_eu(kWavesShade, kWavesShade))) void wf_shade(WfArgs a, HrptPathTracerConstants cb, uint32_t parity, int bounce, int lastBounce)
@@ -903,6 +927,86 @@
 __global__ __launch_bounds__(kBlock) __attribute__((amdgpu_waves_per_eu(kWavesShade, kWavesShade))) void wf_shade_lt(WfArgs a, HrptPathTracerConstants cb, uint32_t parity, int bounce, int lastBounce)
 {
     shade_paths<MAXL, SIMPLE, PRIMARY, true>(a, cb, parity, bounce, lastBounce);
+}
+
+template <int DEPTH>
+__global__ __launch_bounds__(kBlock) __attribute__((amdgpu_waves_per_eu(kWavesShade, kWavesShade))) void wf_bounce0(WfArgs a, HrptPathTracerConstants cb, int lastBounce)
+{
+    extern __shared__ __attribute__((aligned(128))) char smem[];
+    using Stack = LdsStack<DEPTH, kExtendLdsStack>;
+    Stack stack; LdsBvh<4> lbvh;
+    const SceneView& s = a.scene;
+    char* const shadeSmem = smem + (size_t)Stack::kRows * kBlock * 4;
+    float* const ring = reinterpret_cast<float*>(shadeSmem) + (size_t)uniform(threadIdx.x >> 6) * kBounce0Ring * kShadeRingFields;
+    const LdsShadeTables ldsTables = copy_shade_tables(shadeSmem + kBounce0RingBytes, a);
+    setup_lds<true, DEPTH, 4>(smem, s, stack, lbvh, bounce0_shade_bytes(shade_table_bytes(s.triCount, a.shadeInstances, a.shadeMaterials)));
+    if (DEPTH > kExtendLdsStack) { stack.spill = a.spill[0] + blockIdx.x * kBlock + threadIdx.x; stack.spillStride = gridDim.x * kBlock; }
+
+    const uint32_t wavesPerBlock = kBlock / 64, lane = lane_id();
+    const uint32_t gw = uniform(blockIdx.x * wavesPerBlock + (threadIdx.x >> 6)), totalWaves = gridDim.x * wavesPerBlock;
+    const bool emptyScene = s.nodeCount == 0 && s.rootLeaf == 0;
+    const PrimaryArgs& pr = *a.primaryArgs;
+    unsigned int nRays = 0;
+    ShadeWave w;
+    for (uint32_t seg = gw; seg < a.numSegments; seg += totalWaves) {
+        const uint32_t cnt = uniform(path_count(a, 0u, seg)), segBase = seg * a.segSize;
+        w.outCount = 0; w.shCount = 0;
+        for (uint32_t next = 0; next < cnt; next += 64u) {
+            const uint32_t take = cnt - next < 64u ? cnt - next : 64u;
+            ShadeLane L; L.valid = lane < take; L.inA = true; L.slot = segBase + next + lane;
+            Ray r; r.o = mk3(0.0f, 0.0f, 0.0f); r.d = mk3(0.0f, 0.0f, 1.0f); r.tmin = 0.0f; r.tmax = 1e10f;
+            uint32_t rng = 0;
+            bool active = L.valid && primary_ray(a, pr, L.slot, r.o, r.d, rng);
+            const bool havePath = active;
+            if (active) ++nRays;
+            Hit best; best.valid = false; best.t = 0.0f; best.inst = 0; best.prim = 0; best.u = 0.0f; best.v = 0.0f; best.opaque = 0; best.tri = 0;
+            float tlim = r.tmax; int sp = 0;
+            const RayShear sh = make_shear(r.d);
+            const f3 inv = traversal_rcp(r.d), noi = slab_origin_term(r.o, inv);
+            const bool finite = (r.d.x == r.d.x && r.d.y == r.d.y && r.d.z == r.d.z);
+            int32_t cur = (!active || emptyScene || !finite) ? kTraversalDone : (s.nodeCount == 0 ? s.rootLeaf : 0);
+            active = cur != kTraversalDone;
+            while (__ballot(active) != 0ull) {
+                if (active) {
+                    while (cur >= 0) {
+                        cur = inner_step(lbvh, cur, noi, inv, r.tmin, tlim, stack, sp);
+                        if ((uint32_t)__popcll(__ballot(cur >= 0)) < a.nodeLoopMin) break;
+                    }
+                    if (cur < 0 && cur != kTraversalDone) {
+                        const uint32_t enc = (uint32_t)(~cur), first = enc >> 2, count = (enc & 3u) + 1u;
+                        for (uint32_t i = 0; i < count; ++i) {
+                            float4 ta, tb, tc; lbvh.tri(first + i, ta, tb, tc);
+                            float t, u, v;
+                            if (tri_test(mk3(ta.x, ta.y, ta.z), mk3(tb.x, tb.y, tb.z), mk3(tc.x, tc.y, tc.z), r, sh, t, u, v)) {
+                                const uint32_t inst = __float_as_uint(ta.w), prim = __float_as_uint(tb.w);
+                                const bool takeHit = !best.valid || key_less(t, inst, prim, best.t, best.inst, best.prim);
+                                best.t = takeHit ? t : best.t; best.u = takeHit ? u : best.u; best.v = takeHit ? v : best.v;
+                                best.inst = takeHit ? inst : best.inst; best.prim = takeHit ? prim : best.prim; best.tri = takeHit ? first + i : best.tri;
+                                best.opaque = takeHit ? (__float_as_uint(tc.w) & 7u) : best.opaque;
+                                best.valid = best.valid || takeHit;
+                                tlim = takeHit ? t : tlim;
+                            }
+                        }
+                        cur = sp == 0 ? kTraversalDone : stack.pop(--sp);
+                    }
+                    active = cur != kTraversalDone;
+                }
+            }
+            L.o = make_float4(pr.cam[0], pr.cam[1], pr.cam[2], 0.0f);
+            L.d = make_float4(r.d.x, r.d.y, r.d.z, __uint_as_float(rng));
+            L.t = make_float4(1.0f, 1.0f, 1.0f, __uint_as_float(L.slot));
+            L.ha = make_float4(best.t, best.u, best.v, __uint_as_float(!havePath ? kNoPathRecord : (best.valid ? (best.tri | ((best.opaque >> 1) << 29)) : 0xFFFFFFFFu)));
+            uint32_t outCountB, shCountB;
+            shade_iteration<1, true, true, kBounce0Ring, true>(a, cb, ldsTables, ring, 0u, 1u, 0, lastBounce, L, segBase, segBase, next + take >= cnt, w, outCountB, shCountB);
+        }
+        if (lane == 0) { a.b.pathCnt[1][seg] = w.outCount; a.b.shadowCnt[seg] = w.shCount; }
+    }
+    block_count_add(&a.counters->closestRays, 0, nRays);
+    __syncthreads();
+    block_count_add(&a.counters->closestRays, 2, nRays);
+    __syncthreads();
+    block_count_add(&a.counters->closestRays, 8, nRays);
+    block_count_add_uniform<3>(a.counters, { 3, 5, 9 }, { w.nEntriesOut, w.nRadiance, w.nEntriesOut });
 }
 
 template <bool DIRONLY>
@@ -1278,15 +1382,25 @@
 
 TreeCounts tree_counts(const SceneView& scene) { return { scene.nodeCount, scene.node4Count, scene.triCount, scene.nodesQ != nullptr, scene.instances != nullptr, 0u, 0u }; }
 
+hipError_t device_cus(WavefrontState& st, uint32_t& cus, std::string& error)
+{
+    if (!st.cus) {
+        hipError_t e; int dev = 0; hipDeviceProp_t prop;
+        if ((e = hipGetDevice(&dev)) != hipSuccess || (e = hipGetDeviceProperties(&prop, dev)) != hipSuccess) { error = "hipGetDeviceProperties"; return e; }
+        st.cus = (uint32_t)prop.multiProcessorCount;
+    }
+    cus = st.cus;
+    return hipSuccess;
+}
+
 }
 
 hipError_t wavefront_trace_rays(WavefrontState& st, const SceneView& scene, const SceneTraits& traits, const HrptRay* rays, HrptRayHit* hits, uint64_t count,
                                 bool shadow, hipStream_t stream, std::string& error)
 {
     if (count == 0) return hipSuccess;
-    hipError_t e; int dev = 0; hipDeviceProp_t prop;
-    if ((e = hipGetDevice(&dev)) != hipSuccess || (e = hipGetDeviceProperties(&prop, dev)) != hipSuccess) { error = "hipGetDeviceProperties"; return e; }
-    const uint32_t cus = (uint32_t)prop.multiProcessorCount;
+    hipError_t e; uint32_t cus = 0;
+    if ((e = device_cus(st, cus, error)) != hipSuccess) return e;
     const TraceRaysPlan p = plan_trace_rays(traits, tree_counts(scene), count, shadow, cus, st.knobs);
     WfTraceArgs a{};
     a.scene = scene; a.rays = rays; a.hits = hits; a.count = count;
@@ -1374,6 +1488,8 @@
         trace -= c.paths * 16;
         shade = shade - c.paths * (path - 16) + c.paths * 16;
         shadow -= c.skipped16 * 16;
+        trace -= c.fusedPaths * 32;
+        shade = shade - c.fusedPaths * 32 + c.fusedEntries * 16;
     }
 }
 
@@ -1424,10 +1540,8 @@
 {
     (void)height;
     if (rect.x1 <= rect.x0 || rect.y1 <= rect.y0 || rect.columns() == 0) return hipSuccess;
-    hipError_t e;
-    int dev = 0; hipDeviceProp_t prop;
-    if ((e = hipGetDevice(&dev)) != hipSuccess || (e = hipGetDeviceProperties(&prop, dev)) != hipSuccess) { error = "hipGetDeviceProperties"; return e; }
-    const uint32_t cus = (uint32_t)prop.multiProcessorCount;
+    hipError_t e; uint32_t cus = 0;
+    if ((e = device_cus(st, cus, error)) != hipSuccess) return e;
     TreeCounts tree = tree_counts(scene);
     tree.instanceCount = st.shadeInstances; tree.materialCount = st.shadeMaterials;
     const RenderPlan& plan = st.plan = plan_render(traits, tree, constants.m_LightCount, cus, st.knobs);
@@ -1539,14 +1653,20 @@
         for (int bounce = 0; bounce < maxBounces; ++bounce) {
             const uint32_t parity = (uint32_t)bounce & 1u;
             const bool timed = st.profile && st.eventsUsed + 8 <= 4096;
-            if (timed) timing_mark(st, stream, 0, true);
             a.primary = (fusedPrimary && bounce == 0) ? 1u : 0u;
-            launch_extend(plan.vE, cus, dim3(batch.gridExtend), stream, a, parity);
-            if (timed) { timing_mark(st, stream, 0, false); timing_mark(st, stream, 1, true); }
+            const bool fusedBounce0 = plan.fusedBounce0 && bounce == 0;
+            if (timed && !fusedBounce0) timing_mark(st, stream, 0, true);
+            if (!fusedBounce0) launch_extend(plan.vE, cus, dim3(batch.gridExtend), stream, a, parity);
+            if (timed) { if (!fusedBounce0) timing_mark(st, stream, 0, false); timing_mark(st, stream, 1, true); }
             if (pendingJoin) { if ((e = hipStreamWaitEvent(stream, st.joinEvents[(size_t)bounce - 1], 0)) != hipSuccess) { error = "hipStreamWaitEvent(join)"; return e; } pendingJoin = false; }
             const int last = bounce + 1 == maxBounces ? 1 : 0;
             const size_t sortLds = (size_t)(kBlock / 64) * ((size_t)5 * a.segSize);
-            if (maxLights > kMaxLights) hipLaunchKernelGGL((wf_shade<0, false>), grid, dim3(kBlock), sortLds, stream, a, cb, parity, bounce, last);
+            if (fusedBounce0) {
+                if (plan.vE.depth <= 16) hipLaunchKernelGGL((wf_bounce0<16>), grid, dim3(kBlock), plan.bounce0LdsBytes, stream, a, cb, last);
+                else if (plan.vE.depth <= 32) hipLaunchKernelGGL((wf_bounce0<32>), grid, dim3(kBlock), plan.bounce0LdsBytes, stream, a, cb, last);
+                else hipLaunchKernelGGL((wf_bounce0<64>), grid, dim3(kBlock), plan.bounce0LdsBytes, stream, a, cb, last);
+            }
+            else if (maxLights > kMaxLights) hipLaunchKernelGGL((wf_shade<0, false>), grid, dim3(kBlock), sortLds, stream, a, cb, parity, bounce, last);
             else if (maxLights > 1) hipLaunchKernelGGL((wf_shade<(int)kMaxLights, false>), grid, dim3(kBlock), sortLds, stream, a, cb, parity, bounce, last);
             else if (plan.simpleScene && plan.shadeLdsTables && a.primary) hipLaunchKernelGGL((wf_shade_lt<1, true, true>), grid, dim3(kBlock), plan.shadeLdsBytes, stream, a, cb, parity, bounce, last);
             else if (plan.simpleScene && plan.shadeLdsTables) hipLaunchKernelGGL((wf_shade_lt<1, true>), grid, dim3(kBlock), plan.shadeLdsBytes, stream, a, cb, parity, bounce, last);
@@ -1599,10 +1719,8 @@
                              float4* const* planes, uint32_t planeMask, uint32_t width, TileRect rect, hipStream_t stream, std::string& error, const MotionArgs* motion)
 {
     if (rect.x1 <= rect.x0 || rect.y1 <= rect.y0 || rect.columns() == 0) return hipSuccess;
-    hipError_t e;
-    int dev = 0; hipDeviceProp_t prop;
-    if ((e = hipGetDevice(&dev)) != hipSuccess || (e = hipGetDeviceProperties(&prop, dev)) != hipSuccess) { error = "hipGetDeviceProperties"; return e; }
-    const uint32_t cus = (uint32_t)prop.multiProcessorCount;
+    hipError_t e; uint32_t cus = 0;
+    if ((e = device_cus(st, cus, error)) != hipSuccess) return e;
     const uint32_t tilesX = rect.columns(), tilesY = (rect.y1 - rect.y0 + 7) / 8;
     const uint64_t pixelsPadded = (uint64_t)tilesX * tilesY * 64;
     const uint64_t capacity = ((pixelsPadded + kMaxSegment - 1) / kMaxSegment) * kMaxSegment;
diff --git a/hobbyrenderer_amd/csrc/pt_wavefront_plan.h b/hobbyrenderer_amd/csrc/pt_wavefront_plan.h
--- a/hobbyrenderer_amd/csrc/pt_wavefront_plan.h
+++ b/hobbyrenderer_amd/csrc/pt_wavefront_plan.h
@@ -38,6 +38,7 @@
     bool noFusedPrimary = false;
     bool noSlimShadow = false;
     int shadeSort = -1;
+    bool noFusedBounce0 = false;
     bool noShadeLdsTables = false;
     int shadowPath = 0;
 };
@@ -63,11 +64,15 @@
 constexpr size_t kCuLdsBytes = 160 * 1024, kShadeLdsMargin = 1024;
 constexpr size_t kShadeLdsPerBlock = kCuLdsBytes / kShadeBlocksPerCu - kShadeLdsMargin;
 constexpr size_t kTriAttrBytes = 80, kInstShadeBytes = 48, kMaterialBytes = 180;
-inline size_t shade_table_bytes(uint32_t triCount, uint32_t instanceCount, uint32_t materialCount)
+constexpr size_t shade_table_bytes(uint32_t triCount, uint32_t instanceCount, uint32_t materialCount)
 {
     const size_t b = (size_t)triCount * kTriAttrBytes + (size_t)instanceCount * kInstShadeBytes + (size_t)materialCount * kMaterialBytes;
     return (b + 15) & ~(size_t)15;
 }
+constexpr uint32_t kBounce0Ring = 32;
+constexpr size_t kBounce0RingBytes = (size_t)(kBlock / 64) * kBounce0Ring * kShadeRingFields * 4;
+static_assert(kBounce0RingBytes % 128 == 0, "the tree copy behind ring and tables starts 128-byte aligned");
+constexpr size_t bounce0_shade_bytes(size_t tableBytes) { return kBounce0RingBytes + ((tableBytes + 127) & ~(size_t)127); }
 enum : int { kShadowOpaque = 0, kShadowBuffered = 1, kShadowResolve = 2, kShadowSlim = 3 };
 
 struct Variant { bool lds = false; int depth = 0, width = 0; size_t ldsBytes = 0; bool twoLevel = false; bool twoLevelCandidates = false; bool quantised = false; };
@@ -106,6 +111,8 @@
     bool shadeLdsTables = false;
     size_t shadeTableBytes = 0;
     size_t shadeLdsBytes = 0;
+    bool fusedBounce0 = false;
+    size_t bounce0LdsBytes = 0;
 };
 struct BatchPlan { uint32_t segSize, numSegments, grid, gridExtend; };
 
@@ -151,6 +158,10 @@
         if (kShadeRingBytes + tables <= kShadeLdsPerBlock) { p.shadeLdsTables = true; p.shadeTableBytes = tables; p.shadeLdsBytes = kShadeRingBytes + tables; }
     }
     p.fusedPrimary = p.simpleScene && !manyLights && maxLights <= kMaxLights && p.vE.width == 4 && !traits.hasMedium && !traits.hasStochasticAlpha && !k.noFusedPrimary;
+    if (p.fusedPrimary && p.shadeLdsTables && p.vE.lds && p.vE.width == 4 && !traits.hasNonOpaque && !manyLights && !k.noFusedBounce0) {
+        const size_t bytes = p.vE.ldsBytes + bounce0_shade_bytes(p.shadeTableBytes);
+        if (bytes <= kShadeLdsPerBlock) { p.fusedBounce0 = true; p.bounce0LdsBytes = bytes; }
+    }
     return p;
 }
 
```
